# ShreyasBhaktharam/RDEIC

Measured on AMD Instinct MI355X. Metric: 512x512 images/sec encode+relay-decode @ fixed bpp; 1/2/4/8 GPU, higher is better.
Workload: dtype bf16; 1 GPU; config 2: global batch 16 (16/GPU) 512x512, 2-step relay DDIM, encode+entropy-code+decode+VAE-decode; global_batch=16, image_size=512, ddim_steps=2, sampler=ddim, parallelism=dp1, codec_sessions_per_gpu=5

## Files before the change

include/rdeic_hip.h:

```cpp
#ifndef RDEIC_HIP_H
#define RDEIC_HIP_H
#include <stddef.h>
#include <stdint.h>
#ifdef __cplusplus
extern "C" {
#endif

int rdeic_version(void);
int rdeic_abi_count(void);

typedef struct rdeic_conv_desc {
  const void* in0;
  const void* in1;
  int32_t c0, c1;
  int32_t ld0, ld1;
  int32_t n, h, w;
  int32_t up2;
  const void* weight;
  int32_t wld;
  const float* bias;
  int32_t cout, kh, kw, stride, pad_t, pad_l;
  int32_t ho, wo;
  const float* gn_ab;
  int32_t gn_silu;
  const float* emb;
  int32_t emb_ld;
  int32_t act;
  float act_param;
  const void* res;
  int32_t res_ld;
  void* out;
  int32_t out_ld;
  int32_t out_mode;
  int32_t dtype;
  int32_t out_f32;
  int32_t batch;
  int64_t in_bs, w_bs, out_bs;
  float* gn_part;
  int32_t gn_hw;
  int32_t reserved;
  const float* ln_rows;
  const float* ln_colsum;
} rdeic_conv_desc;

int rdeic_conv2d(const rdeic_conv_desc* d, void* stream);
int rdeic_conv2d_tile(const rdeic_conv_desc* d, int32_t tile, void* stream);
int rdeic_conv2d_splitk(const rdeic_conv_desc* d, int32_t splits, float* ws, size_t ws_floats, void* stream);
int rdeic_set_conv_path(int32_t path);
int rdeic_set_conv_option(int32_t key, int32_t value);

size_t rdeic_groupnorm_ws_floats(int32_t n, int32_t hw, int32_t c);
size_t rdeic_groupnorm_parts_floats(int64_t rows, int32_t c, int32_t hw);
int rdeic_groupnorm_parts_ab(const float* p0, int32_t c0, const float* p1, int32_t c1, int32_t n, int32_t hw,
                             int32_t groups, float eps, const float* gamma, const float* beta, float* ab,
                             void* stream);
int rdeic_groupnorm_stats(const void* x0, int32_t c0, int32_t ld0, const void* x1, int32_t c1, int32_t ld1,
                          int32_t n, int32_t hw, int32_t groups, float eps, const float* gamma, const float* beta,
                          float* ab, float* ws, int32_t dtype, void* stream);
int rdeic_groupnorm_parts_apply(const float* p0, int32_t c0, const float* p1, int32_t c1, const void* x0, int32_t ld0,
                                const void* x1, int32_t ld1, int32_t n, int32_t hw, int32_t groups, float eps,
                                const float* gamma, const float* beta, int32_t silu, float* ab, void* y, int32_t yld,
                                void* stream);
int rdeic_groupnorm_apply(const void* x, int32_t n, int32_t hw, int32_t c, int32_t ld, const float* ab,
                          int32_t ab_c, int32_t silu, float out_mul, void* y, int32_t yld, int32_t dtype,
                          void* stream);
int rdeic_layernorm(const void* x, int32_t rows, int32_t c, int32_t ld, const float* gamma, const float* beta,
                    float eps, void* y, int32_t yld, int32_t dtype, void* stream);

int rdeic_attention(const void* q, int32_t ldq, const void* k, int32_t ldk, const void* v, int32_t ldv,
                    void* o, int32_t ldo, int32_t batch, int32_t heads, int32_t lq, int32_t lk, int32_t dh,
                    float scale, int32_t kv_bcast, int32_t dtype, void* stream);
int rdeic_softmax_rows(const float* s, int64_t rows, int32_t cols, float scale, void* p, int32_t dtype, void* stream);
int rdeic_transpose(const void* in, int32_t rows, int32_t cols, int32_t ldin, void* out, int32_t ldout,
                    int32_t batch, int64_t in_bs, int64_t out_bs, int32_t dtype, void* stream);

int rdeic_geglu(const void* in, int32_t rows, int32_t c, int32_t ldin, void* out, int32_t ldout,
                int32_t dtype, void* stream);
int rdeic_nchw_to_nhwc(const float* in, int32_t n, int32_t c, int32_t h, int32_t w, float mul, float add,
                       void* out, int32_t ld, int32_t dtype, void* stream);
int rdeic_nhwc_to_nchw(const void* in, int32_t n, int32_t c, int32_t h, int32_t w, int32_t ld, float mul,
                       float add, float* out, int32_t dtype, void* stream);
int rdeic_axpby(const float* x, const float* z, int32_t n_img, int32_t per_img, const float* a,
                const float* b, float* y, void* stream);
int rdeic_timestep_embedding(const int64_t* t, const float* freqs, int32_t n, int32_t dim, float* out, void* stream);
int rdeic_ddim_step(const float* x, const float* e, int64_t count, float c_sq1m, float c_sqa, float c_sqap,
                    float c_dir, float* xp, float* x0, void* stream);
int rdeic_cfg_combine(const float* e_cond, const float* e_uncond, int64_t count, float scale, float* out,
                      void* stream);
int rdeic_spaced_step(const float* x, const float* e, const float* noise, int64_t count, float a, float b, float c1,
                      float c2, float s, float* xp, float* x0, void* stream);
int rdeic_silu_f32(const float* x, float* y, int64_t count, void* stream);
int rdeic_image_u8_to_nhwc(const uint8_t* img, int32_t n, int32_t h, int32_t w, void* out, int32_t ld,
                           int32_t dtype, void* stream);
int rdeic_nhwc_to_image_u8(const void* x, int32_t n, int32_t h, int32_t w, int32_t ld, uint8_t* img,
                           int32_t dtype, void* stream);
int rdeic_image_mse(const uint8_t* a, const uint8_t* b, int32_t n, int64_t per_img, float* out, void* stream);
int rdeic_fill_uniform(float* out, int64_t count, uint64_t seed, float scale, float offset, void* stream);
int rdeic_pack_conv_weight(const float* w, int32_t cout, int32_t cin, int32_t kh, int32_t kw, void* out,
                           int32_t wld, int32_t dtype, void* stream);
int rdeic_cast(const void* in, int32_t in_dtype, void* out, int32_t out_dtype, int64_t count, void* stream);

int rdeic_ckbd_encode(const void* y, int32_t yld, const void* params, int32_t pld, int32_t n, int32_t hy,
                      int32_t wy, int32_t c, int32_t phase, const float* scale_table, int32_t levels,
                      float scale_bound, int32_t* sym, int32_t* idx, int64_t img_stride, int64_t off,
                      void* yhat, int32_t yhld, void* anchor_out, int32_t ald, int32_t dtype, void* stream);
int rdeic_ckbd_indexes(const void* params, int32_t pld, int32_t n, int32_t hy, int32_t wy, int32_t c,
                       int32_t phase, const float* scale_table, int32_t levels, float scale_bound,
                       int32_t* idx, int64_t img_stride, int64_t off, int32_t dtype, void* stream);
int rdeic_ckbd_dequant(const int32_t* sym, const void* params, int32_t pld, int32_t n, int32_t hy,
                       int32_t wy, int32_t c, int32_t phase, int64_t img_stride, int64_t off, void* yhat,
                       int32_t yhld, void* anchor_out, int32_t ald, int32_t dtype, void* stream);
int rdeic_vq_argmin(const float* dot, const float* zn, const float* en, int32_t rows, int32_t ncode, int32_t* idx,
                    void* stream);
int rdeic_gather_rows(const float* table, int32_t ld_table, const int32_t* idx, int32_t rows, int32_t dim,
                      void* out, int32_t ld_out, int32_t dtype, void* stream);
int rdeic_row_sqnorm(const void* x, int32_t rows, int32_t dim, int32_t ld, float* out, int32_t dtype,
                     void* stream);

size_t rdeic_image_ssim_ws_floats(int32_t n, int32_t h, int32_t w, int32_t levels);
int rdeic_image_ssim(const uint8_t* a, const uint8_t* b, int32_t n, int32_t h, int32_t w, int32_t levels, float* ws,
                     size_t ws_floats, float* out, void* stream);

int rdeic_pmf_to_quantized_cdf(const float* pmf, int32_t n, int32_t precision, uint32_t* cdf_out);
int rdeic_build_gaussian_tables(const float* pmf, const int32_t* pmf_len, int32_t levels, int32_t pmf_ld,
                                int32_t* cdf, int32_t cdf_ld, int32_t* cdf_len, void* reserved);

int rdeic_rans_encode(const int32_t* sym, const int32_t* idx, size_t n, const int32_t* cdf, int32_t cdf_ld,
                      const int32_t* cdf_len, const int32_t* offset, int32_t levels, uint8_t* out, size_t cap,
                      size_t* out_len);
int rdeic_rans_encode_batch(int32_t count, const int32_t* sym, const int32_t* idx, size_t n_per,
                            size_t stride, const int32_t* cdf, int32_t cdf_ld, const int32_t* cdf_len,
                            const int32_t* offset, int32_t levels, uint8_t* out, size_t cap_per,
                            size_t* out_len, int32_t threads);
void* rdeic_rans_enc_tables_create(const int32_t* cdf, int32_t cdf_ld, const int32_t* cdf_len,
                                   const int32_t* offset, int32_t levels);
void rdeic_rans_enc_tables_destroy(void* tables);
int rdeic_rans_encode_batch_t(const void* tables, int32_t count, const int32_t* sym, const int32_t* idx,
                              size_t n_per, size_t stride, uint8_t* out, size_t cap_per, size_t* out_len,
                              int32_t threads);
int rdeic_rans_enc_quotient(const void* tables, int32_t row, int32_t value, uint64_t x, uint64_t* q);
void* rdeic_rans_dec_open(const uint8_t* data, size_t len);
int rdeic_rans_decode(void* handle, const int32_t* idx, size_t n, const int32_t* cdf, int32_t cdf_ld,
                      const int32_t* cdf_len, const int32_t* offset, int32_t levels, int32_t* out);
int rdeic_rans_decode_batch(int32_t count, void** handles, const int32_t* idx, size_t n_per, size_t stride,
                            const int32_t* cdf, int32_t cdf_ld, const int32_t* cdf_len, const int32_t* offset,
                            int32_t levels, int32_t* out, int32_t threads);
void rdeic_rans_dec_close(void* handle);

int rdeic_ac_encode(const int16_t* sym, size_t n, const int16_t* cdf_row, int32_t lp, uint8_t* out,
                    size_t cap, size_t* out_len);
int rdeic_ac_decode(const uint8_t* data, size_t len, size_t n, const int16_t* cdf_row, int32_t lp,
                    int16_t* out);
int rdeic_ac_uniform_cdf(int32_t codebook_size, int16_t* cdf_row);

#define RDEIC_PROF_CONV 0
#define RDEIC_PROF_ATTN 1
#define RDEIC_PROF_ATTN_SMALL 2
#define RDEIC_PROF_GN_STATS 3
#define RDEIC_PROF_GN_APPLY 4
#define RDEIC_PROF_GEMM 5
#define RDEIC_PROF_ATTN_D512 6
#define RDEIC_PROF_CONV_BYTES 7
int rdeic_prof_start(int32_t capacity, int32_t every);
int rdeic_prof_read_keys(int32_t kind, int64_t* keys, int64_t* launches, double* work, double* ms, int32_t cap);
#define RDEIC_COUNT_HALO_CONV 0
#define RDEIC_COUNT_GN_APPLY 1
#define RDEIC_COUNT_LAYERNORM 2
#define RDEIC_COUNT_HALO_SMALL 3
#define RDEIC_COUNT_LN_FUSED 4
#define RDEIC_COUNT_SPLITK 5
#define RDEIC_COUNT_EDGE 6
#define RDEIC_COUNT_GN_PARTS_APPLY 7
#define RDEIC_COUNT_KINDS 8
int64_t rdeic_launch_count(int32_t kind);
int rdeic_layernorm_rowstats(const void* x, int32_t rows, int32_t c, int32_t ld, float eps, float* ms,
                             void* stream);
int rdeic_launch_count_reset(void);
int rdeic_prof_stop(void);
int rdeic_prof_read(int32_t kind, int64_t* launches, double* work, double* ms);

typedef struct rdeic_gemm_desc {
  const void* a;
  int64_t a_bs1, a_bs2, a_sm, a_sk;
  const void* b;
  int64_t b_bs1, b_bs2, b_sk, b_sn;
  void* c;
  int64_t c_bs1, c_bs2, c_sm;
  int32_t batch, nb2, m, n, k, ksplit, dtype, c_f32;
  float alpha, beta;
  float* rsum;
  int64_t rsum_bs;
} rdeic_gemm_desc;
int rdeic_gemm_strided(const rdeic_gemm_desc* d, void* stream);
int rdeic_pack_conv_weight_dgrad(const float* w, int32_t cout, int32_t cin, int32_t kh, int32_t kw, void* out,
                                 int32_t wld, int32_t to_bf16, void* stream);
typedef struct rdeic_pack_job {
  const float* w;
  void* out;
  int64_t start;
  int32_t cout, cin, kh, kw, wld, mode;
// ... 73 lines not shown
```

rdeic_amd/_lib.py:

```python
from __future__ import annotations

import ctypes as C
import os
import threading

_HERE = os.path.dirname(os.path.abspath(__file__))
LIB_PATH = os.environ.get("RDEIC_LIB") or os.path.join(_HERE, "lib", "librdeic_hip.so")

EINVAL, ENOSPC, EBADMSG, ELAUNCH = -22, -28, -74, -5
_ERRNAMES = {EINVAL: "EINVAL (bad argument/shape)", ENOSPC: "ENOSPC (output capacity)",
             EBADMSG: "EBADMSG (corrupt or truncated bitstream)", ELAUNCH: "kernel launch failure"}


class RdeicError(RuntimeError):
    def __init__(self, fn: str, code: int):
        super().__init__(f"{fn} failed: {code} {_ERRNAMES.get(code, '')}")
        self.code = code


class BitstreamError(RdeicError, ValueError):
    """Corrupt / truncated bitstream (the reference's 'decode failure')."""


class ConvDesc(C.Structure):
    _fields_ = [
        ("in0", C.c_void_p), ("in1", C.c_void_p),
        ("c0", C.c_int32), ("c1", C.c_int32), ("ld0", C.c_int32), ("ld1", C.c_int32),
        ("n", C.c_int32), ("h", C.c_int32), ("w", C.c_int32), ("up2", C.c_int32),
        ("weight", C.c_void_p), ("wld", C.c_int32),
        ("bias", C.c_void_p),
        ("cout", C.c_int32), ("kh", C.c_int32), ("kw", C.c_int32), ("stride", C.c_int32),
        ("pad_t", C.c_int32), ("pad_l", C.c_int32),
        ("ho", C.c_int32), ("wo", C.c_int32),
        ("gn_ab", C.c_void_p), ("gn_silu", C.c_int32),
        ("emb", C.c_void_p), ("emb_ld", C.c_int32),
        ("act", C.c_int32), ("act_param", C.c_float),
        ("res", C.c_void_p), ("res_ld", C.c_int32),
        ("out", C.c_void_p), ("out_ld", C.c_int32), ("out_mode", C.c_int32),
        ("dtype", C.c_int32), ("out_f32", C.c_int32),
        ("batch", C.c_int32), ("in_bs", C.c_int64), ("w_bs", C.c_int64), ("out_bs", C.c_int64),
        ("gn_part", C.c_void_p), ("gn_hw", C.c_int32), ("reserved", C.c_int32),
        ("ln_rows", C.c_void_p), ("ln_colsum", C.c_void_p),
    ]


class GemmDesc(C.Structure):
    _fields_ = [
        ("a", C.c_void_p), ("a_bs1", C.c_int64), ("a_bs2", C.c_int64), ("a_sm", C.c_int64), ("a_sk", C.c_int64),
        ("b", C.c_void_p), ("b_bs1", C.c_int64), ("b_bs2", C.c_int64), ("b_sk", C.c_int64), ("b_sn", C.c_int64),
        ("c", C.c_void_p), ("c_bs1", C.c_int64), ("c_bs2", C.c_int64), ("c_sm", C.c_int64),
        ("batch", C.c_int32), ("nb2", C.c_int32), ("m", C.c_int32), ("n", C.c_int32), ("k", C.c_int32),
        ("ksplit", C.c_int32), ("dtype", C.c_int32), ("c_f32", C.c_int32),
        ("alpha", C.c_float), ("beta", C.c_float), ("rsum", C.c_void_p), ("rsum_bs", C.c_int64),
    ]


_p, _i32, _i64, _u64, _f, _sz = C.c_void_p, C.c_int32, C.c_int64, C.c_uint64, C.c_float, C.c_size_t

PROTOTYPES = {
    "rdeic_version": (C.c_int, []),
    "rdeic_abi_count": (C.c_int, []),
    "rdeic_conv2d": (C.c_int, [C.POINTER(ConvDesc), _p]),
    "rdeic_conv2d_splitk": (C.c_int, [C.POINTER(ConvDesc), _i32, _p, C.c_size_t, _p]),
    "rdeic_conv2d_tile": (C.c_int, [C.POINTER(ConvDesc), _i32, _p]),
    "rdeic_prof_start": (C.c_int, [_i32, _i32]),
    "rdeic_prof_stop": (C.c_int, []),
    "rdeic_launch_count": (C.c_int64, [_i32]),
    "rdeic_launch_count_reset": (C.c_int, []),
    "rdeic_layernorm_rowstats": (C.c_int, [C.c_void_p, _i32, _i32, _i32, C.c_float, C.c_void_p, C.c_void_p]),
    "rdeic_prof_read": (C.c_int, [_i32, C.POINTER(C.c_int64), C.POINTER(C.c_double), C.POINTER(C.c_double)]),
    "rdeic_prof_read_keys": (C.c_int, [_i32, C.POINTER(C.c_int64), C.POINTER(C.c_int64), C.POINTER(C.c_double),
                                       C.POINTER(C.c_double), _i32]),
    "rdeic_groupnorm_ws_floats": (_sz, [_i32, _i32, _i32]),
    "rdeic_groupnorm_stats": (C.c_int, [_p, _i32, _i32, _p, _i32, _i32, _i32, _i32, _i32, _f, _p, _p, _p, _p,
                                        _i32, _p]),
    "rdeic_groupnorm_apply": (C.c_int, [_p, _i32, _i32, _i32, _i32, _p, _i32, _i32, _f, _p, _i32, _i32, _p]),
    "rdeic_set_conv_path": (C.c_int, [_i32]),
    "rdeic_set_conv_option": (C.c_int, [_i32, _i32]),
    "rdeic_layernorm": (C.c_int, [_p, _i32, _i32, _i32, _p, _p, _f, _p, _i32, _i32, _p]),
    "rdeic_softmax_rows": (C.c_int, [_p, _i64, _i32, _f, _p, _i32, _p]),
    "rdeic_transpose": (C.c_int, [_p, _i32, _i32, _i32, _p, _i32, _i32, _i64, _i64, _i32, _p]),
    "rdeic_attention": (C.c_int, [_p, _i32, _p, _i32, _p, _i32, _p, _i32, _i32, _i32, _i32, _i32, _i32, _f,
                                  _i32, _i32, _p]),
    "rdeic_geglu": (C.c_int, [_p, _i32, _i32, _i32, _p, _i32, _i32, _p]),
    "rdeic_nchw_to_nhwc": (C.c_int, [_p, _i32, _i32, _i32, _i32, _f, _f, _p, _i32, _i32, _p]),
    "rdeic_nhwc_to_nchw": (C.c_int, [_p, _i32, _i32, _i32, _i32, _i32, _f, _f, _p, _i32, _p]),
    "rdeic_axpby": (C.c_int, [_p, _p, _i32, _i32, _p, _p, _p, _p]),
    "rdeic_timestep_embedding": (C.c_int, [_p, _p, _i32, _i32, _p, _p]),
    "rdeic_ddim_step": (C.c_int, [_p, _p, _i64, _f, _f, _f, _f, _p, _p, _p]),
    "rdeic_spaced_step": (C.c_int, [_p, _p, _p, _i64, _f, _f, _f, _f, _f, _p, _p, _p]),
    "rdeic_cfg_combine": (C.c_int, [_p, _p, _i64, _f, _p, _p]),
    "rdeic_silu_f32": (C.c_int, [_p, _p, _i64, _p]),
    "rdeic_image_u8_to_nhwc": (C.c_int, [_p, _i32, _i32, _i32, _p, _i32, _i32, _p]),
    "rdeic_nhwc_to_image_u8": (C.c_int, [_p, _i32, _i32, _i32, _i32, _p, _i32, _p]),
    "rdeic_image_mse": (C.c_int, [_p, _p, _i32, _i64, _p, _p]),
    "rdeic_fill_uniform": (C.c_int, [_p, _i64, _u64, _f, _f, _p]),
    "rdeic_pack_conv_weight": (C.c_int, [_p, _i32, _i32, _i32, _i32, _p, _i32, _i32, _p]),
    "rdeic_cast": (C.c_int, [_p, _i32, _p, _i32, _i64, _p]),
    "rdeic_ckbd_encode": (C.c_int, [_p, _i32, _p, _i32, _i32, _i32, _i32, _i32, _i32, _p, _i32, _f, _p, _p,
                                    _i64, _i64, _p, _i32, _p, _i32, _i32, _p]),
    "rdeic_ckbd_indexes": (C.c_int, [_p, _i32, _i32, _i32, _i32, _i32, _i32, _p, _i32, _f, _p, _i64, _i64,
                                     _i32, _p]),
    "rdeic_ckbd_dequant": (C.c_int, [_p, _p, _i32, _i32, _i32, _i32, _i32, _i32, _i64, _i64, _p, _i32, _p,
                                     _i32, _i32, _p]),
    "rdeic_vq_argmin": (C.c_int, [_p, _p, _p, _i32, _i32, _p, _p]),
    "rdeic_gather_rows": (C.c_int, [_p, _i32, _p, _i32, _i32, _p, _i32, _i32, _p]),
    "rdeic_row_sqnorm": (C.c_int, [_p, _i32, _i32, _i32, _p, _i32, _p]),
    "rdeic_pmf_to_quantized_cdf": (C.c_int, [_p, _i32, _i32, _p]),
    "rdeic_build_gaussian_tables": (C.c_int, [_p, _p, _i32, _i32, _p, _i32, _p, _p]),
    "rdeic_rans_encode": (C.c_int, [_p, _p, _sz, _p, _i32, _p, _p, _i32, _p, _sz, C.POINTER(_sz)]),
    "rdeic_rans_encode_batch": (C.c_int, [_i32, _p, _p, _sz, _sz, _p, _i32, _p, _p, _i32, _p, _sz, _p, _i32]),
    "rdeic_image_ssim_ws_floats": (C.c_size_t, [_i32, _i32, _i32, _i32]),
    "rdeic_image_ssim": (C.c_int, [_p, _p, _i32, _i32, _i32, _i32, _p, C.c_size_t, _p, _p]),
    "rdeic_groupnorm_parts_floats": (C.c_size_t, [_i64, _i32, _i32]),
    "rdeic_groupnorm_parts_ab": (C.c_int, [_p, _i32, _p, _i32, _i32, _i32, _i32, _f, _p, _p, _p, _p]),
    "rdeic_groupnorm_parts_apply": (C.c_int, [_p, _i32, _p, _i32, _p, _i32, _p, _i32, _i32, _i32, _i32, _f, _p, _p,
                                              _i32, _p, _p, _i32, _p]),
    "rdeic_rans_enc_tables_create": (_p, [_p, _i32, _p, _p, _i32]),
    "rdeic_rans_enc_tables_destroy": (None, [_p]),
    "rdeic_rans_encode_batch_t": (C.c_int, [_p, _i32, _p, _p, _sz, _sz, _p, _sz, _p, _i32]),
    "rdeic_rans_enc_quotient": (C.c_int, [_p, _i32, _i32, C.c_uint64, C.POINTER(C.c_uint64)]),
    "rdeic_rans_dec_open": (_p, [_p, _sz]),
    "rdeic_rans_decode": (C.c_int, [_p, _p, _sz, _p, _i32, _p, _p, _i32, _p]),
    "rdeic_rans_decode_batch": (C.c_int, [_i32, _p, _p, _sz, _sz, _p, _i32, _p, _p, _i32, _p, _i32]),
    "rdeic_rans_dec_close": (None, [_p]),
    "rdeic_ac_encode": (C.c_int, [_p, _sz, _p, _i32, _p, _sz, C.POINTER(_sz)]),
    "rdeic_ac_decode": (C.c_int, [_p, _sz, _sz, _p, _i32, _p]),
    "rdeic_ac_uniform_cdf": (C.c_int, [_i32, _p]),
    "rdeic_gemm_strided": (C.c_int, [C.POINTER(GemmDesc), _p]),
    "rdeic_pack_conv_weight_dgrad": (C.c_int, [_p, _i32, _i32, _i32, _i32, _p, _i32, _i32, _p]),
    "rdeic_pack_batch": (C.c_int, [_p, _i32, _i64, _i32, _i32, _p]),
    "rdeic_zero_insert2": (C.c_int, [_p, _i32, _i32, _i32, _i32, _i32, _p, _i32, _i32, _p]),
    "rdeic_sum_pool2": (C.c_int, [_p, _i32, _i32, _i32, _i32, _i32, _p, _i32, _i32, _p]),
    "rdeic_pixel_unshuffle2": (C.c_int, [_p, _i32, _i32, _i32, _i32, _i32, _p, _i32, _i32, _p]),
    "rdeic_im2col": (C.c_int, [_p, _i32, _i32, _i32, _i32, _i32, _i32, _i32, _i32, _i32, _i32, _i32, _i32, _i32, _p,
                               _i64, _i32, _p]),
    "rdeic_wgrad_finalize": (C.c_int, [_p, _i32, _i32, _i32, _i32, _i32, _p, _i32, _p, _p, _p]),
    "rdeic_col_sum_ws_floats": (_sz, [_i64, _i32, _i32]),
    "rdeic_col_sum": (C.c_int, [_p, _i64, _i32, _i32, _i32, _p, _i32, _p, _sz, _i32, _p]),
    "rdeic_act_fwd": (C.c_int, [_p, _i64, _i32, _i32, _p, _i32, _i32, _f, _p, _i32, _i32, _p]),
    "rdeic_act_bwd": (C.c_int, [_p, _i32, _p, _i32, _i64, _i32, _i32, _f, _p, _i32, _i32, _p]),
    "rdeic_gn_train_ws_doubles": (_sz, [_i32, _i32, _i32]),
    "rdeic_gn_train_fwd": (C.c_int, [_p, _i32, _i32, _i32, _i32, _i32, _f, _p, _p, _p, _p, _p, _i32, _p]),
    "rdeic_gn_train_bwd": (C.c_int, [_p, _i32, _p, _i32, _i32, _i32, _i32, _i32, _p, _p, _p, _i32, _p, _i32, _p, _p,
                                     _i32, _p, _p, _i32, _p]),
    "rdeic_gn_train_bwd_res": (C.c_int, [_p, _i32, _p, _i32, _i32, _i32, _i32, _i32, _p, _p, _p, _i32, _p, _i32, _p,
                                         _i32, _p, _p, _i32, _p, _p, _i32, _p]),
    "rdeic_layernorm_bwd_ws_floats": (_sz, [_i64, _i32]),
    "rdeic_layernorm_bwd": (C.c_int, [_p, _i32, _i64, _i32, _p, _f, _p, _i32, _p, _i32, _p, _p, _i32, _p, _sz, _i32,
                                      _p]),
    "rdeic_layernorm_bwd_res": (C.c_int, [_p, _i32, _i64, _i32, _p, _f, _p, _i32, _p, _i32, _p, _i32, _p, _p, _i32, _p,
                                          _sz, _i32, _p]),
    "rdeic_softmax_bwd_rows": (C.c_int, [_p, _p, _i64, _i32, _f, _p, _i32, _p]),
    "rdeic_geglu_bwd": (C.c_int, [_p, _i32, _i64, _i32, _p, _i32, _p, _i32, _i32, _p]),
    "rdeic_ckbd_train_anchor": (C.c_int, [_p, _i32, _p, _i32, _i32, _i32, _i32, _i32, _p, _i32, _i32, _p]),
    "rdeic_ckbd_mask": (C.c_int, [_p, _i32, _i32, _i32, _i32, _i32, _i32, _p, _i32, _i32, _p]),
    "rdeic_ckbd_train_ws_doubles": (_sz, [_i32, _i32, _i32, _i32]),
    "rdeic_ckbd_train_lik": (C.c_int, [_p, _i32, _p, _i32, _p, _i32, _p, _i32, _i32, _i32, _i32, _p, _i32, _p, _p,
                                       _i32, _p]),
    "rdeic_ckbd_train_lik_bwd": (C.c_int, [_p, _i32, _p, _i32, _p, _i32, _p, _i32, _i32, _i32, _i32, _p, _p, _i32, _p,
                                           _i32, _p, _i32, _p, _i32, _i32, _p]),
    "rdeic_vq_train": (C.c_int, [_p, _p, _p, _p, _p, _i32, _i32, _i32, _p, _p, _f, _f, _f, _p, _p, _p, _p]),
    "rdeic_vq_z_grad": (C.c_int, [_p, _p, _p, _i64, _p, _f, _p, _i32, _p]),
    "rdeic_scale_dev": (C.c_int, [_p, _i64, _p, _p, _i32, _p]),
    "rdeic_adamw": (C.c_int, [_p, _p, _p, _p, _i64, _f, _f, _f, _f, _f, _i32, _p]),
    "rdeic_adamw_dev": (C.c_int, [_p, _p, _p, _p, _i64, _f, _f, _f, _f, _f, _p, _p]),
}

_lib = None
_lock = threading.Lock()


def load() -> C.CDLL:
    global _lib
    if _lib is not None:
        return _lib
    with _lock:
        if _lib is not None:
            return _lib
        if not os.path.exists(LIB_PATH):
            raise ImportError(f"librdeic_hip.so not built at {LIB_PATH}; run `make` (or __graft_entry__.build()).")
        import torch
        lib = C.CDLL(LIB_PATH, mode=C.RTLD_GLOBAL)
        for name, (res, args) in PROTOTYPES.items():
            fn = getattr(lib, name)
            fn.restype = res
            fn.argtypes = args
        _lib = lib
    return _lib


def check(name: str, rc: int) -> None:
    if rc != 0:
        if rc == EBADMSG:
            raise BitstreamError(name, rc)
        raise RdeicError(name, rc)


RECORDER = None


def call(name: str, *args, tag=None) -> None:
    fn = getattr(load(), name)
    if RECORDER is not None:
        RECORDER.append((name, fn, args, tag))
    rc = fn(*args)
    check(name, rc)
```

rdeic_amd/csrc/coders.cpp:

```cpp
#include <stdint.h>
#include <string.h>

#include <algorithm>
#include <atomic>
#include <condition_variable>
#include <functional>
#include <mutex>
#include <cmath>
#include <new>
#include <stdexcept>
#include <thread>
#include <vector>

#include "../../include/rdeic_hip.h"

#define RDEIC_OK 0
#define RDEIC_EINVAL (-22)
#define RDEIC_ENOSPC (-28)
#define RDEIC_EBADMSG (-74)

namespace {

constexpr int kPrecision = 16;
constexpr uint32_t kBypassBits = 4;
// ... 244 lines not shown
  }
  return d->bad ? RDEIC_EBADMSG : RDEIC_OK;
}

class WorkerPool {
 public:
  static WorkerPool& get() {
    thread_local WorkerPool* p = new WorkerPool();
    return *p;
  }
  void run(int32_t count, int32_t threads, const std::function<void(int32_t)>& f) {
    std::lock_guard<std::mutex> job(job_mu_);
    int32_t helpers = std::max(0, std::min(threads, count) - 1);
    while ((int32_t)workers_.size() < helpers) {
      const int32_t id = (int32_t)workers_.size();
      try {
        workers_.reserve(workers_.size() + 1);
        std::thread(&WorkerPool::loop, this, id).detach();
      } catch (...) {
        helpers = (int32_t)workers_.size();
        break;
      }
      workers_.push_back(id);
    }
    {
      std::lock_guard<std::mutex> lk(mu_);
      fn_ = &f;
      count_ = count;
      next_.store(0);
      helpers_ = helpers;
      active_ = helpers;
      ++gen_;
    }
    cv_.notify_all();
    work();
    std::unique_lock<std::mutex> lk(mu_);
    done_cv_.wait(lk, [&] { return active_ == 0; });
    fn_ = nullptr;
  }

 private:
  void work() {
    for (;;) {
      const int32_t i = next_.fetch_add(1);
      if (i >= count_) break;
      (*fn_)(i);
    }
  }
  void loop(int32_t id) {
    uint64_t seen = 0;
    for (;;) {
      {
        std::unique_lock<std::mutex> lk(mu_);
        cv_.wait(lk, [&] { return gen_ != seen; });
        seen = gen_;
        if (id >= helpers_) continue;
      }
      work();
      std::lock_guard<std::mutex> lk(mu_);
      if (--active_ == 0) done_cv_.notify_all();
    }
  }

  std::mutex job_mu_, mu_;
  std::condition_variable cv_, done_cv_;
  std::vector<int32_t> workers_;
  const std::function<void(int32_t)>* fn_ = nullptr;
  std::atomic<int32_t> next_{0};
  int32_t count_ = 0, active_ = 0, helpers_ = 0;
  uint64_t gen_ = 0;
};

template <typename F>
int guard(F&& f) noexcept {
  try {
    return f();
  } catch (const std::bad_alloc&) {
    return RDEIC_ENOSPC;
  } catch (...) {
    return RDEIC_EINVAL;
  }
}

template <typename F>
void parallel_for(int32_t count, int32_t threads, F&& f) {
  if (threads <= 1 || count <= 1) {
    for (int32_t i = 0; i < count; ++i) f(i);
    return;
  }
  const std::function<void(int32_t)> fn = f;
  WorkerPool::get().run(count, threads, fn);
}

struct BitWriter {
  uint8_t* out;
  size_t cap;
  size_t len = 0;
  uint8_t cache = 0;
  int count = 0;
  bool overflow = false;
  void put(int bit) {
    cache = (uint8_t)((cache << 1) | (bit & 1));
    if (++count == 8) {
      if (len < cap) out[len] = cache; else overflow = true;
      ++len;
      count = 0;
      cache = 0;
    }
  }
  void put_with_pending(int bit, uint64_t& pending) {
    put(bit);
    while (pending > 0) { put(!bit); --pending; }
  }
  void flush() {
    while (count > 0) put(0);
  }
};

struct BitReader {
  const uint8_t* in;
  size_t n;
  size_t ptr = 0;
  uint8_t cache = 0;
  int cached = 0;
  void get(uint32_t& value) {
    if (cached == 0) {
      if (ptr == n) { value <<= 1; return; }
      cache = in[ptr++];
      cached = 8;
    }
    value = (value << 1) | ((cache >> (cached - 1)) & 1);
    --cached;
  }
};

inline uint16_t binsearch_u16(const uint16_t* cdf, uint16_t target, uint16_t max_sym) {
  uint16_t left = 0, right = (uint16_t)(max_sym + 1);
  while (left + 1 < right) {
    const uint16_t m = (uint16_t)((left + right) / 2);
    const uint16_t v = cdf[m];
    if (v < target) left = m;
    else if (v > target) right = m;
    else return m;
  }
  return left;
}

}

extern "C" {

int rdeic_version(void) { return 1; }

int rdeic_abi_count(void) { return 93; }

static int pmf_to_quantized_cdf_impl(const float* pmf, int32_t n, int32_t precision, uint32_t* cdf_out) {
  if (!pmf || !cdf_out || n <= 0 || precision <= 0 || precision > 24) return RDEIC_EINVAL;
  for (int32_t i = 0; i < n; ++i)
    if (!(pmf[i] >= 0.f) || !std::isfinite(pmf[i])) return RDEIC_EINVAL;
  const uint32_t one = 1u << precision;
  std::vector<uint32_t> cdf((size_t)n + 1);
  cdf[0] = 0;
  for (int32_t i = 0; i < n; ++i) cdf[i + 1] = (uint32_t)std::round(pmf[i] * (float)one);
  uint64_t total = 0;
  for (uint32_t v : cdf) total += v;
  if (total == 0) return RDEIC_EINVAL;
  for (auto& v : cdf) v = (uint32_t)(((uint64_t)one * v) / total);
  for (size_t i = 1; i < cdf.size(); ++i) cdf[i] += cdf[i - 1];
  cdf.back() = one;
  const int32_t m = (int32_t)cdf.size();
  for (int32_t i = 0; i < m - 1; ++i) {
    if (cdf[i] == cdf[i + 1]) {
      uint32_t best_freq = ~0u;
      int32_t best = -1;
      for (int32_t j = 0; j < m - 1; ++j) {
        const uint32_t f = cdf[j + 1] - cdf[j];
        if (f > 1 && f < best_freq) { best_freq = f; best = j; }
      }
      if (best < 0) return RDEIC_EINVAL;
      if (best < i) {
        for (int32_t j = best + 1; j <= i; ++j) cdf[j]--;
      } else {
        for (int32_t j = i + 1; j <= best; ++j) cdf[j]++;
      }
    }
  }
  memcpy(cdf_out, cdf.data(), cdf.size() * sizeof(uint32_t));
  return RDEIC_OK;
}

int rdeic_pmf_to_quantized_cdf(const float* pmf, int32_t n, int32_t precision, uint32_t* cdf_out) {
  return guard([&] { return pmf_to_quantized_cdf_impl(pmf, n, precision, cdf_out); });
}

static int build_gaussian_tables_impl(const float* pmf, const int32_t* pmf_len, int32_t levels, int32_t pmf_ld,
                                      int32_t* cdf, int32_t cdf_ld, int32_t* cdf_len) {
  if (!pmf || !pmf_len || !cdf || !cdf_len || levels <= 0) return RDEIC_EINVAL;
  std::vector<float> row;
  std::vector<uint32_t> q;
  for (int32_t i = 0; i < levels; ++i) {
    const int32_t L = pmf_len[i];
    if (L <= 0 || L + 1 > pmf_ld || L + 2 > cdf_ld) return RDEIC_EINVAL;
    row.assign(pmf + (size_t)i * pmf_ld, pmf + (size_t)i * pmf_ld + L + 1);
    q.assign((size_t)L + 2, 0u);
    int rc = pmf_to_quantized_cdf_impl(row.data(), L + 1, kPrecision, q.data());
    if (rc) return rc;
    int32_t* out = cdf + (size_t)i * cdf_ld;
    for (int32_t j = 0; j < cdf_ld; ++j) out[j] = j < L + 2 ? (int32_t)q[j] : 0;
    cdf_len[i] = L + 2;
  }
  return RDEIC_OK;
}

int rdeic_build_gaussian_tables(const float* pmf, const int32_t* pmf_len, int32_t levels, int32_t pmf_ld, int32_t* cdf,
                                int32_t cdf_ld, int32_t* cdf_len, void* reserved) {
  (void)reserved;
  return guard([&] { return build_gaussian_tables_impl(pmf, pmf_len, levels, pmf_ld, cdf, cdf_ld, cdf_len); });
}

int rdeic_rans_encode(const int32_t* sym, const int32_t* idx, size_t n, const int32_t* cdf, int32_t cdf_ld,
                      const int32_t* cdf_len, const int32_t* offset, int32_t levels, uint8_t* out, size_t cap,
                      size_t* out_len) {
  if ((!sym || !idx) && n) return RDEIC_EINVAL;
  if (!cdf || !cdf_len || !offset || !out || !out_len || levels <= 0) return RDEIC_EINVAL;
  return guard([&] {
    std::vector<RansSym> syms;
    std::vector<uint32_t> words;
    return rans_encode_impl(sym, idx, n, cdf, cdf_ld, cdf_len, offset, levels, out, cap, out_len, syms, words);
  });
}

int rdeic_rans_encode_batch(int32_t count, const int32_t* sym, const int32_t* idx, size_t n_per, size_t stride,
                            const int32_t* cdf, int32_t cdf_ld, const int32_t* cdf_len, const int32_t* offset,
                            int32_t levels, uint8_t* out, size_t cap_per, size_t* out_len, int32_t threads) {
  if (count <= 0 || !sym || !idx || !out || !out_len) return RDEIC_EINVAL;
  return guard([&] {
    std::vector<int> rc(count, 0);
    parallel_for(count, threads, [&](int32_t i) {
      rc[i] = guard([&] {
        std::vector<RansSym> syms;
        std::vector<uint32_t> words;
        return rans_encode_impl(sym + i * stride, idx + i * stride, n_per, cdf, cdf_ld, cdf_len, offset, levels,
                                out + i * cap_per, cap_per, &out_len[i], syms, words);
      });
    });
    for (int v : rc)
      if (v) return v;
    return (int)RDEIC_OK;
  });
}

void* rdeic_rans_enc_tables_create(const int32_t* cdf, int32_t cdf_ld, const int32_t* cdf_len, const int32_t* offset,
                                   int32_t levels) {
  if (!cdf || !cdf_len || !offset || levels <= 0 || cdf_ld < 2) return nullptr;
  EncTables* T = new (std::nothrow) EncTables();
  if (!T) return nullptr;
  try {
    T->levels = levels;
    T->row_off.resize(levels);
    T->max_value.resize(levels);
    T->offset.assign(offset, offset + levels);
    size_t total = 0;
    for (int32_t ci = 0; ci < levels; ++ci) {
      const int32_t len = cdf_len[ci];
      if (len < 2 || len > cdf_ld) throw std::invalid_argument("cdf_len");
      T->row_off[ci] = (int32_t)total;
      T->max_value[ci] = len - 2;
      total += (size_t)len - 1;
    }
    T->sym.resize(total);
    for (int32_t ci = 0; ci < levels; ++ci) {
      const int32_t* row = cdf + (size_t)ci * cdf_ld;
      for (int32_t v = 0; v <= T->max_value[ci]; ++v) {
        const int32_t start = row[v], freq = row[v + 1] - row[v];
        if (start < 0 || freq <= 0 || start + freq > (1 << kPrecision)) throw std::invalid_argument("cdf row");
        T->sym[(size_t)T->row_off[ci] + v] = make_enc_sym((uint32_t)start, (uint32_t)freq);
      }
    }
  } catch (...) {
    delete T;
    return nullptr;
  }
  return T;
}

void rdeic_rans_enc_tables_destroy(void* tables) { delete (EncTables*)tables; }

int rdeic_rans_encode_batch_t(const void* tables, int32_t count, const int32_t* sym, const int32_t* idx, size_t n_per,
                              size_t stride, uint8_t* out, size_t cap_per, size_t* out_len, int32_t threads) {
  if (!tables || count <= 0 || ((!sym || !idx) && n_per) || !out || !out_len) return RDEIC_EINVAL;
  const EncTables& T = *(const EncTables*)tables;
  return guard([&] {
    std::vector<int> rc(count, 0);
    parallel_for(count, threads, [&](int32_t i) {
      rc[i] = guard([&] {
        thread_local std::vector<uint32_t> buf;
        return rans_encode_tab_impl(T, sym + i * stride, idx + i * stride, n_per, out + i * cap_per, cap_per,
                                    &out_len[i], buf);
      });
    });
    for (int v : rc)
      if (v) return v;
    return (int)RDEIC_OK;
  });
}

int rdeic_rans_enc_quotient(const void* tables, int32_t row, int32_t value, uint64_t x, uint64_t* q) {
// ... 151 lines not shown
```

rdeic_amd/csrc/conv_common.h:

```cpp
#pragma once
#include "common.h"
#include "../../include/rdeic_hip.h"
#include "prof.h"

namespace rdeic_conv {

struct ConvArgs {
  const char* in0; const char* in1;
  int c0, c1, ld0, ld1;
  int n, h, w, up2;
  const char* weight; int wld;
  const float* bias;
  int cout, kh, kw, stride, pad_t, pad_l, ho, wo;
  const float* gn_ab; int gn_silu;
  const float* emb; int emb_ld;
  int act; float act_param;
  const char* res; int res_ld;
  char* out; int out_ld, out_mode;
  int out_f32;
  int M, cin, ktot, nk;
  long in_bs, w_bs, out_bs;
  int batch;
  int epi_vec;
  int splits, kper;
  float* gn_part;
  int gn_row0;
  int gn_hw;
  const float* ln_rows;
  const float* ln_cs;
};

__device__ __forceinline__ float ln_fold(const ConvArgs& a, int m, int n, float v) {
  const float2 ms = reinterpret_cast<const float2*>(a.ln_rows)[m];
  return ms.y * (v - ms.x * a.ln_cs[n]);
}

constexpr int ROWB = 144;

template <typename T, bool SWZ = true> __host__ __device__ constexpr int tile_rowb() { return (sizeof(T) == 2 && SWZ) ? 128 : ROWB; }
template <typename T, bool SWZ = true> __device__ __forceinline__ int chunk_key(int r) {
  if constexpr (sizeof(T) == 2 && SWZ) return (((r >> 3) & 1) << 1) | (((r >> 1) & 1) << 2);
  return 0;
}
template <typename T, int BM, int BN, bool SWZ = true> __host__ __device__ constexpr int conv_lds_bytes() {
  return (2 * (BM + BN) * tile_rowb<T, SWZ>() > (BM / 2) * (BN + 4) * 4 || sizeof(T) != 2)
             ? 2 * (BM + BN) * tile_rowb<T, SWZ>()
             : (BM / 2) * (BN + 4) * 4;
}

template <typename T> struct MmaTraits;
template <> struct MmaTraits<bf16> {
  static constexpr int BK = 64;
  static constexpr int EPC = 8;
};
template <> struct MmaTraits<float> {
  static constexpr int BK = 32;
  static constexpr int EPC = 4;
};

__device__ __forceinline__ float apply_act(float v, int act, float p) {
  if (act == 1) return v >= 0.f ? v : v * p;
  if (act == 2) return gelu_f(v);
  if (act == 3) return silu_f(v);
  return v;
}

__device__ __forceinline__ uint4 ld16(const char* p) { return *reinterpret_cast<const uint4*>(p); }

template <typename T>
__device__ __forceinline__ uint4 gn_apply_chunk(uint4 raw, const float* ab, int silu) {
  constexpr int E = MmaTraits<T>::EPC;
  T v[E];
  *reinterpret_cast<uint4*>(v) = raw;
#pragma unroll
  for (int e = 0; e < E; ++e) {
    float x = to_f32(v[e]);
    x = x * ab[2 * e] + ab[2 * e + 1];
    if (silu) x = silu_f(x);
    v[e] = from_f32<T>(x);
  }
  return *reinterpret_cast<uint4*>(v);
}

__host__ __device__ __forceinline__ bool epi_vec_ok(const ConvArgs& a) {
  if (a.out_mode == 2) return (a.cout % 8) == 0 && (a.out_ld % 4) == 0 && ((uintptr_t)a.out % 8) == 0;
  return a.out_mode == 0 && (a.cout % 8) == 0 && (a.out_ld % 8) == 0 && ((uintptr_t)a.out % 16) == 0 &&
         (!a.res || ((a.res_ld % 8) == 0 && ((uintptr_t)a.res % 16) == 0));
}

struct RowsFrom {
  int m0;
  __device__ __forceinline__ int operator()(int r) const { return m0 + r; }
};

template <int BM, int BN, int WGM, int WGN, int NT, int P = 2, class RowMap = RowsFrom, bool PF = true>
__device__ __forceinline__ void epilogue_vec(const f32x4 (&acc)[BM / WGM / 16][BN / WGN / 16], const ConvArgs& a,
                                             int m0, int n0, int wm, int wn, int lane, int tid, char* lds,
                                             RowMap rmap = RowMap{0}) {
  if constexpr (__is_same(RowMap, RowsFrom)) rmap.m0 = m0;
  constexpr int WTM = BM / WGM, WTN = BN / WGN;
  constexpr int TM = WTM / 16, TN = WTN / 16;
  constexpr int HM = TM / P;
  constexpr int PR = BM / P;
  constexpr int SDW = BN + 4;
  constexpr int CPR = BN / 8;
  static_assert(TM % P == 0, "P passes");
  const int lr = lane & 15, lq = lane >> 4;
  float* L = reinterpret_cast<float*>(lds);
  const int hw_o = a.ho * a.wo;
  const bool of32 = a.out_f32;
  const bool st = a.gn_part != nullptr;
  constexpr int NU = ((BM / 64) * BN + NT - 1) / NT;
  float sg[NU][4], qg[NU][4];
#pragma unroll
  for (int u = 0; u < NU; ++u)
#pragma unroll
    for (int g = 0; g < 4; ++g) sg[u][g] = qg[u][g] = 0.f;
  constexpr int NCH = (PR * CPR + NT - 1) / NT;
  constexpr int NPF = !PF ? 0 : NCH < 2 ? NCH : 2;
  constexpr bool HOIST = PF && (NT % CPR) == 0;
  auto bar = []() { asm volatile("s_waitcnt lgkmcnt(0)\n\ts_barrier" ::: "memory"); };
  float4 bh[2] = {float4{0.f, 0.f, 0.f, 0.f}, float4{0.f, 0.f, 0.f, 0.f}}, chh[2] = {bh[0], bh[0]};
  if constexpr (HOIST) {
    const int nn = n0 + (tid % CPR) * 8;
    if (nn < a.cout) {
      if (a.bias) {
        bh[0] = *reinterpret_cast<const float4*>(a.bias + nn);
        bh[1] = *reinterpret_cast<const float4*>(a.bias + nn + 4);
      }
      if (a.ln_rows) {
        chh[0] = *reinterpret_cast<const float4*>(a.ln_cs + nn);
        chh[1] = *reinterpret_cast<const float4*>(a.ln_cs + nn + 4);
      }
    }
  }
#pragma unroll
  for (int p = 0; p < P; ++p) {
    uint4 rpf[NPF > 0 ? NPF : 1];
    float2 lpf[NPF > 0 ? NPF : 1];
#pragma unroll
    for (int k = 0; k < NPF; ++k) {
      const int c = tid + k * NT;
      const int pr = c / CPR, cc = c - pr * CPR;
      const int wmr = pr / (WTM / P), wr = pr - wmr * (WTM / P);
      const int m = rmap(wmr * WTM + p * (WTM / P) + wr);
      const int nn = n0 + cc * 8;
      const bool ok = c < PR * CPR && m < a.M && nn < a.cout;
      rpf[k] = uint4{0u, 0u, 0u, 0u};
      lpf[k] = float2{0.f, 0.f};
      if (ok) {
        if (a.res && !of32 && a.out_mode != 2)
          rpf[k] = *reinterpret_cast<const uint4*>(reinterpret_cast<const bf16*>(a.res) + (long)m * a.res_ld + nn);
        if (a.ln_rows) lpf[k] = reinterpret_cast<const float2*>(a.ln_rows)[m];
      }
    }
    bar();
#pragma unroll
    for (int ii = 0; ii < HM; ++ii)
#pragma unroll
      for (int r = 0; r < 4; ++r) {
        const int pr = wm * (WTM / P) + ii * 16 + lq * 4 + r;
#pragma unroll
        for (int j = 0; j < TN; ++j) L[pr * SDW + wn * WTN + j * 16 + lr] = acc[p * HM + ii][j][r];
      }
    bar();
#pragma unroll
    for (int k = 0; k < NCH; ++k) {
      const int c = tid + k * NT;
      if (c >= PR * CPR) continue;
      const int pr = c / CPR, cc = c - pr * CPR;
      const int wmr = pr / (WTM / P), wr = pr - wmr * (WTM / P);
      const int m = rmap(wmr * WTM + p * (WTM / P) + wr);
      const int nn = n0 + cc * 8;
      if (m >= a.M || nn >= a.cout) continue;
      float v[8];
      const float4 x0 = *reinterpret_cast<const float4*>(L + pr * SDW + cc * 8);
      const float4 x1 = *reinterpret_cast<const float4*>(L + pr * SDW + cc * 8 + 4);
      v[0] = x0.x; v[1] = x0.y; v[2] = x0.z; v[3] = x0.w; v[4] = x1.x; v[5] = x1.y; v[6] = x1.z; v[7] = x1.w;
      if (a.ln_rows) {
        const float2 ms = k < NPF ? lpf[k < NPF ? k : 0] : reinterpret_cast<const float2*>(a.ln_rows)[m];
        float4 c0 = chh[0], c1 = chh[1];
        if constexpr (!HOIST) {
          c0 = *reinterpret_cast<const float4*>(a.ln_cs + nn);
          c1 = *reinterpret_cast<const float4*>(a.ln_cs + nn + 4);
        }
        const float cs[8] = {c0.x, c0.y, c0.z, c0.w, c1.x, c1.y, c1.z, c1.w};
        const f32x2 nm = {-ms.x, -ms.x}, rs = {ms.y, ms.y};
#pragma unroll
        for (int e = 0; e < 8; e += 2) {
          const f32x2 r = rs * pk_fma(nm, f32x2{cs[e], cs[e + 1]}, f32x2{v[e], v[e + 1]});
          v[e] = r.x;
          v[e + 1] = r.y;
        }
      }
      if (a.bias) {
        float4 b0 = bh[0], b1 = bh[1];
        if constexpr (!HOIST) {
          b0 = *reinterpret_cast<const float4*>(a.bias + nn);
          b1 = *reinterpret_cast<const float4*>(a.bias + nn + 4);
        }
        const float bs[8] = {b0.x, b0.y, b0.z, b0.w, b1.x, b1.y, b1.z, b1.w};
#pragma unroll
        for (int e = 0; e < 8; e += 2) {
          const f32x2 r = f32x2{v[e], v[e + 1]} + f32x2{bs[e], bs[e + 1]};
          v[e] = r.x;
          v[e + 1] = r.y;
        }
      }
      if (a.emb) {
        const float* em = a.emb + (long)(m / hw_o) * a.emb_ld + nn;
#pragma unroll
        for (int e = 0; e < 8; ++e) v[e] += em[e];
      }
#pragma unroll
      for (int e = 0; e < 8; ++e) v[e] = apply_act(v[e], a.act, a.act_param);
      if (a.out_mode == 2) {
        bf16 gv[4];
#pragma unroll
        for (int e = 0; e < 4; e += 2) {
          const f32x2 xv = {to_f32(from_f32<bf16>(v[e])), to_f32(from_f32<bf16>(v[e + 1]))};
          const f32x2 gt = {to_f32(from_f32<bf16>(v[4 + e])), to_f32(from_f32<bf16>(v[5 + e]))};
          const f32x2 r = xv * gelu_fast2(gt);
          gv[e] = from_f32<bf16>(r.x);
          gv[e + 1] = from_f32<bf16>(r.y);
        }
        *reinterpret_cast<uint2*>(reinterpret_cast<bf16*>(a.out) + (long)m * a.out_ld + (nn >> 1)) =
            *reinterpret_cast<uint2*>(gv);
        continue;
      }
      if (a.res) {
        if (of32) {
          const float4 r0 = *reinterpret_cast<const float4*>(reinterpret_cast<const float*>(a.res) + (long)m * a.res_ld + nn);
          const float4 r1 = *reinterpret_cast<const float4*>(reinterpret_cast<const float*>(a.res) + (long)m * a.res_ld + nn + 4);
          v[0] += r0.x; v[1] += r0.y; v[2] += r0.z; v[3] += r0.w; v[4] += r1.x; v[5] += r1.y; v[6] += r1.z; v[7] += r1.w;
        } else {
          bf16 rv[8];
          *reinterpret_cast<uint4*>(rv) =
              k < NPF ? rpf[k < NPF ? k : 0]
                      : *reinterpret_cast<const uint4*>(reinterpret_cast<const bf16*>(a.res) + (long)m * a.res_ld + nn);
#pragma unroll
          for (int e = 0; e < 8; ++e) v[e] += to_f32(rv[e]);
        }
      }
      if (of32) {
        float* o = reinterpret_cast<float*>(a.out) + (long)m * a.out_ld + nn;
        *reinterpret_cast<float4*>(o) = make_float4(v[0], v[1], v[2], v[3]);
        *reinterpret_cast<float4*>(o + 4) = make_float4(v[4], v[5], v[6], v[7]);
        if (st) {
          *reinterpret_cast<float4*>(L + pr * SDW + cc * 8) = make_float4(v[0], v[1], v[2], v[3]);
          *reinterpret_cast<float4*>(L + pr * SDW + cc * 8 + 4) = make_float4(v[4], v[5], v[6], v[7]);
        }
      } else {
        bf16 ov[8];
#pragma unroll
        for (int e = 0; e < 8; ++e) ov[e] = from_f32<bf16>(v[e]);
        *reinterpret_cast<uint4*>(reinterpret_cast<bf16*>(a.out) + (long)m * a.out_ld + nn) = *reinterpret_cast<uint4*>(ov);
        if (st) {
          *reinterpret_cast<float4*>(L + pr * SDW + cc * 8) =
              make_float4(to_f32(ov[0]), to_f32(ov[1]), to_f32(ov[2]), to_f32(ov[3]));
          *reinterpret_cast<float4*>(L + pr * SDW + cc * 8 + 4) =
              make_float4(to_f32(ov[4]), to_f32(ov[5]), to_f32(ov[6]), to_f32(ov[7]));
        }
      }
    }
    if constexpr ((WTM == 32 || WTM == 64) && (WTM / P) % 16 == 0) {
      if (st) {
        bar();
#pragma unroll
        for (int u = 0; u < NU; ++u) {
        const int b = (tid + u * NT) / BN, j = (tid + u * NT) % BN;
        if (b < BM / 64) {
          constexpr int WPB = 64 / WTM;
#pragma unroll
          for (int w = 0; w < WPB; ++w) {
            const int wmr = b * WPB + w;
#pragma unroll
            for (int k = 0; k < (WTM / P) / 16; ++k) {
              const int off = w * WTM + p * (WTM / P) + k * 16;
              const float* col = L + (wmr * (WTM / P) + k * 16) * SDW + j;
              const int nv = a.M - (rmap(b * 64) + off);
              float s1 = 0.f, s2 = 0.f;
              if (nv >= 16) {
                float y[16];
#pragma unroll
                for (int r = 0; r < 16; ++r) y[r] = col[r * SDW];
#pragma unroll
                for (int r = 0; r < 16; ++r) { s1 += y[r]; s2 = fmaf(y[r], y[r], s2); }
              } else {
                for (int r = 0; r < nv; ++r) { const float y = col[r * SDW]; s1 += y; s2 = fmaf(y, y, s2); }
              }
              sg[u][off >> 4] = s1;
              qg[u][off >> 4] = s2;
            }
          }
        }
        }
      }
    }
  }
  if constexpr ((WTM == 32 || WTM == 64) && (WTM / P) % 16 == 0) {
    if (st) {
#pragma unroll
      for (int u = 0; u < NU; ++u) {
        const int b = (tid + u * NT) / BN, j = (tid + u * NT) % BN;
        const int nn = n0 + j;
        if (b < BM / 64 && nn < a.cout && rmap(b * 64) < a.M) {
          float* pp = a.gn_part + 4 + ((long)((a.gn_row0 + rmap(b * 64)) / 64) * a.cout + nn) * 2;
          pp[0] = ((sg[u][0] + sg[u][1]) + sg[u][2]) + sg[u][3];
          pp[1] = ((qg[u][0] + qg[u][1]) + qg[u][2]) + qg[u][3];
        }
      }
      if (tid == 0 && rmap(0) == 0 && n0 == 0) reinterpret_cast<int*>(a.gn_part)[0] = 64;
    }
  }
}

template <int BM, int BN, int WGM, int NT, int P>
constexpr bool stats_tile_ok() {
  constexpr int WTM = BM / WGM;
  return (WTM == 32 || WTM == 64) && (WTM / P) % 16 == 0;
}

template <int BM, int BN, int WGM, int WGN, int NT, int P>
__device__ __forceinline__ void epilogue_geglu(const f32x4 (&acc)[BM / WGM / 16][BN / WGN / 16], const ConvArgs& a,
                                               int m0, int n0, int wm, int wn, int lane, int tid, char* lds) {
  constexpr int WTM = BM / WGM, WTN = BN / WGN;
  constexpr int TM = WTM / 16, TN = WTN / 16;
  constexpr int HM = TM / P;
  constexpr int PR = BM / P;
  constexpr int SDW = BN + 4;
  constexpr int DPR = BN / 16;
  constexpr int ND = (PR * DPR + NT - 1) / NT;
  constexpr int NPF = ND < 2 ? ND : 2;
  constexpr bool HOIST = (NT % DPR) == 0;
  static_assert(TM % P == 0 && BN % 16 == 0, "P passes, chunk pairs");
  const int lr = lane & 15, lq = lane >> 4;
  float* L = reinterpret_cast<float*>(lds);
  auto bar = []() { asm volatile("s_waitcnt lgkmcnt(0)\n\ts_barrier" ::: "memory"); };
  auto row_of = [&](int d, int p) {
    const int pr = d / DPR;
    const int wmr = pr / (WTM / P), wr = pr - wmr * (WTM / P);
    return m0 + wmr * WTM + p * (WTM / P) + wr;
  };
  float4 bh[4], chh[4];
#pragma unroll
  for (int q = 0; q < 4; ++q) bh[q] = chh[q] = float4{0.f, 0.f, 0.f, 0.f};
  if constexpr (HOIST) {
    const int nn = n0 + (tid % DPR) * 16;
    if (nn < a.cout) {
#pragma unroll
      for (int q = 0; q < 4; ++q) {
        if (a.bias) bh[q] = *reinterpret_cast<const float4*>(a.bias + nn + 4 * q);
        if (a.ln_rows) chh[q] = *reinterpret_cast<const float4*>(a.ln_cs + nn + 4 * q);
      }
    }
  }
#pragma unroll
  for (int p = 0; p < P; ++p) {
    float2 lpf[NPF];
#pragma unroll
    for (int k = 0; k < NPF; ++k) {
      const int d = tid + k * NT;
      const int m = row_of(d, p);
      lpf[k] = float2{0.f, 0.f};
      if (a.ln_rows && d < PR * DPR && m < a.M) lpf[k] = reinterpret_cast<const float2*>(a.ln_rows)[m];
    }
    bar();
#pragma unroll
    for (int ii = 0; ii < HM; ++ii)
#pragma unroll
      for (int r = 0; r < 4; ++r) {
        const int pr = wm * (WTM / P) + ii * 16 + lq * 4 + r;
#pragma unroll
        for (int j = 0; j < TN; ++j) L[pr * SDW + wn * WTN + j * 16 + lr] = acc[p * HM + ii][j][r];
      }
    bar();
#pragma unroll
    for (int k = 0; k < ND; ++k) {
      const int d = tid + k * NT;
      if (d >= PR * DPR) continue;
      const int pr = d / DPR, cq = d - pr * DPR;
      const int m = row_of(d, p);
      const int nn = n0 + cq * 16;
      if (m >= a.M || nn >= a.cout) continue;
      float v[16];
#pragma unroll
      for (int q = 0; q < 4; ++q) {
        const float4 x = *reinterpret_cast<const float4*>(L + pr * SDW + cq * 16 + 4 * q);
        v[4 * q] = x.x; v[4 * q + 1] = x.y; v[4 * q + 2] = x.z; v[4 * q + 3] = x.w;
      }
      if (a.ln_rows) {
        const float2 ms = k < NPF ? lpf[k < NPF ? k : 0] : reinterpret_cast<const float2*>(a.ln_rows)[m];
        const f32x2 nm = {-ms.x, -ms.x}, rs = {ms.y, ms.y};
#pragma unroll
        for (int q = 0; q < 4; ++q) {
          const float4 c = HOIST ? chh[q] : *reinterpret_cast<const float4*>(a.ln_cs + nn + 4 * q);
          const float cs[4] = {c.x, c.y, c.z, c.w};
#pragma unroll
          for (int e = 0; e < 4; e += 2) {
            const f32x2 r = rs * pk_fma(nm, f32x2{cs[e], cs[e + 1]}, f32x2{v[4 * q + e], v[4 * q + e + 1]});
            v[4 * q + e] = r.x;
            v[4 * q + e + 1] = r.y;
          }
        }
      }
      if (a.bias) {
#pragma unroll
        for (int q = 0; q < 4; ++q) {
          const float4 b = HOIST ? bh[q] : *reinterpret_cast<const float4*>(a.bias + nn + 4 * q);
          const f32x2 r0 = f32x2{v[4 * q], v[4 * q + 1]} + f32x2{b.x, b.y};
          const f32x2 r1 = f32x2{v[4 * q + 2], v[4 * q + 3]} + f32x2{b.z, b.w};
          v[4 * q] = r0.x; v[4 * q + 1] = r0.y; v[4 * q + 2] = r1.x; v[4 * q + 3] = r1.y;
        }
      }
#pragma unroll
      for (int e = 0; e < 16; ++e) v[e] = apply_act(v[e], a.act, a.act_param);
      bf16 gv[8];
#pragma unroll
      for (int h = 0; h < 2; ++h)
#pragma unroll
        for (int e = 0; e < 4; e += 2) {
          const f32x2 xv = {to_f32(from_f32<bf16>(v[8 * h + e])), to_f32(from_f32<bf16>(v[8 * h + e + 1]))};
          const f32x2 gt = {to_f32(from_f32<bf16>(v[8 * h + 4 + e])), to_f32(from_f32<bf16>(v[8 * h + 5 + e]))};
          const f32x2 r = xv * gelu_fast2(gt);
          gv[4 * h + e] = from_f32<bf16>(r.x);
          gv[4 * h + e + 1] = from_f32<bf16>(r.y);
        }
      *reinterpret_cast<uint4*>(reinterpret_cast<bf16*>(a.out) + (long)m * a.out_ld + (nn >> 1)) =
          *reinterpret_cast<uint4*>(gv);
    }
  }
}

constexpr unsigned kOOB = 0x80000000u;

template <int N>
__device__ __forceinline__ void wait_vm() {
  asm volatile("s_waitcnt vmcnt(%0)" ::"n"(N) : "memory");
}

__device__ __forceinline__ int dma_key(int r) { return (((r >> 3) & 1) << 1) | (((r >> 1) & 1) << 2); }

typedef __attribute__((address_space(3))) void* lds_ptr_t;

__device__ __forceinline__ void dma16(__amdgpu_buffer_rsrc_t rs, char* lds_dst, unsigned voff, int soff) {
  __builtin_amdgcn_raw_ptr_buffer_load_lds(rs, (lds_ptr_t)lds_dst, 16, (int)voff, soff, 0, 0);
}

#ifdef RDEIC_HALO_STAMPS
__device__ unsigned long long* g_halo_stamps;
#define HALO_STAMP(k)                                                                      \
  do {                                                                                     \
    if (threadIdx.x == 0) g_halo_stamps[(long)blockIdx.x * 8 + (k)] = __builtin_amdgcn_s_memtime(); \
  } while (0)
#else
#define HALO_STAMP(k) do {} while (0)
#endif

__device__ __forceinline__ void wait_vm_rt(int n) {
  switch (n) {
    case 0: wait_vm<0>(); break;
    case 1: wait_vm<1>(); break;
    case 2: wait_vm<2>(); break;
    case 3: wait_vm<3>(); break;
    case 4: wait_vm<4>(); break;
    case 5: wait_vm<5>(); break;
    case 6: wait_vm<6>(); break;
    default: wait_vm<7>(); break;
  }
}

extern int g_conv_path, g_epi_vec, g_swz, g_force_tile, g_dma, g_halo, g_halo8, g_edge;

int make_args(const rdeic_conv_desc* d, ConvArgs& a, bool& vec);
bool dma_ok(const rdeic_conv_desc* d, const ConvArgs& a, unsigned& b0, unsigned& b1, unsigned& bw);
int launch_dma_auto(const ConvArgs& a, unsigned b0, unsigned b1, unsigned bw, hipStream_t s, int tile,
                    int gn_hw = 0, bool* fused = nullptr);
int dma_grouped(const rdeic_conv_desc* d, int tile, hipStream_t s, bool* fused = nullptr);
bool halo_ok(const rdeic_conv_desc* d, const ConvArgs& a);
int launch_halo(const rdeic_conv_desc* d, ConvArgs a, hipStream_t s, bool* fused);
int launch_edge(const rdeic_conv_desc* d, const ConvArgs& a, hipStream_t s, bool* fused);
}
```

rdeic_amd/csrc/conv_dma.hip:

```cpp
#include "conv_common.h"

namespace rdeic_conv {

template <int TM, int TN, int WTM, int WTN>
__device__ __forceinline__ void epilogue_scalar(const f32x4 (&acc)[TM][TN], const ConvArgs& a, int m0, int n0, int wm,
                                                int wn, int lane) {
  if (a.out_mode == 2) return;
  const int lrow = lane & 15, lq = lane >> 4;
  const int hw_o = a.ho * a.wo;
  const bool of32 = a.out_f32;
#pragma unroll
  for (int i = 0; i < TM; ++i) {
#pragma unroll
    for (int r = 0; r < 4; ++r) {
      const int m = m0 + wm * WTM + i * 16 + lq * 4 + r;
      if (m >= a.M) continue;
      const int img = m / hw_o;
      int oy = 0, ox = 0;
      if (a.out_mode == 1) { const int rem = m - img * hw_o; oy = rem / a.wo; ox = rem - oy * a.wo; }
#pragma unroll
      for (int j = 0; j < TN; ++j) {
        const int nn = n0 + wn * WTN + j * 16 + lrow;
        if (nn >= a.cout) continue;
        float v = acc[i][j][r];
        if (a.ln_rows) v = ln_fold(a, m, nn, v);
        if (a.bias) v += a.bias[nn];
        if (a.emb) v += a.emb[(long)img * a.emb_ld + nn];
        v = apply_act(v, a.act, a.act_param);
        long oidx, ridx;
        if (a.out_mode == 1) {
          const int c = nn >> 2, dy = (nn >> 1) & 1, dx = nn & 1;
          const long p = ((long)img * (2 * a.ho) + (2 * oy + dy)) * (2 * a.wo) + (2 * ox + dx);
          oidx = p * a.out_ld + c;
          ridx = p * a.res_ld + c;
        } else {
          oidx = (long)m * a.out_ld + nn;
          ridx = (long)m * a.res_ld + nn;
        }
        if (a.res) v += of32 ? reinterpret_cast<const float*>(a.res)[ridx] : to_f32(reinterpret_cast<const bf16*>(a.res)[ridx]);
        if (of32) reinterpret_cast<float*>(a.out)[oidx] = v;
        else reinterpret_cast<bf16*>(a.out)[oidx] = from_f32<bf16>(v);
      }
    }
  }
}

template <int BM, int BN, int WGM, int WGN, int S, int EP, bool GEG = false>
__device__ __forceinline__ void conv_dma_body(ConvArgs a, int tiles_n, unsigned bytes0, unsigned bytes1,
                                              unsigned bytesw) {
  constexpr int KB = 64;
  constexpr int NW = WGM * WGN, NT = NW * 64;
  constexpr int RB = KB * 2;
  constexpr int RPI = 1024 / RB;
  constexpr int LPR = RB / 16;
  constexpr int KSUB = KB / 32;
  constexpr int A_BYTES = BM * RB, STAGE = (BM + BN) * RB;
  constexpr int AI = BM / NW / RPI, BI = BN / NW / RPI;
  constexpr int PER = AI + BI;
  constexpr int WTM = BM / WGM, WTN = BN / WGN;
  constexpr int TM = WTM / 16, TN = WTN / 16;
  static_assert(AI >= 1 && BI >= 1 && AI * RPI * NW == BM && BI * RPI * NW == BN, "tile / wave split");
  static_assert(S >= 2 && S <= 4 && PER * (S - 2) <= 63, "ring");

  extern __shared__ __attribute__((aligned(16))) char lds[];
  HALO_STAMP(0);

  int kt_begin = 0, kt_end = a.nk;
  if (a.splits > 1) {
    const int z = blockIdx.z;
    kt_begin = min(a.nk, z * a.kper);
    kt_end = min(a.nk, kt_begin + a.kper);
    a.out += (long)z * a.M * a.out_ld * 4;
  } else if (gridDim.z > 1) {
    const long z = blockIdx.z;
    a.in0 += z * a.in_bs * 2; a.in1 += z * a.in_bs * 2;
    a.weight += z * a.w_bs * 2;
    a.out += z * a.out_bs * (a.out_f32 ? 4 : 2);
  }
  const int nwg = gridDim.x, orig = blockIdx.x;
  const int xcd = orig & 7, q = nwg >> 3, rr = nwg & 7;
  const int wgid = (xcd < rr ? xcd * (q + 1) : rr * (q + 1) + (xcd - rr) * q) + (orig >> 3);
  const int mt = wgid / tiles_n, nt = wgid - mt * tiles_n;
  const int m0 = mt * BM, n0 = nt * BN;

  const int tid = threadIdx.x, lane = tid & 63;
  const int wave = __builtin_amdgcn_readfirstlane(tid >> 6);
  const int wm = wave / WGN, wn = wave - (wave / WGN) * WGN;
  const int g = lane / LPR, sl = lane % LPR;
  const int ce = sl ^ (((g >> 1) & 1) << 2);
  const int hw_o = a.ho * a.wo;
  const int hin = a.up2 ? 2 * a.h : a.h, win = a.up2 ? 2 * a.w : a.w;

  const __amdgpu_buffer_rsrc_t rs0 = __builtin_amdgcn_make_buffer_rsrc((void*)a.in0, (short)0, (int)bytes0, 0x00020000);
  const __amdgpu_buffer_rsrc_t rs1 = __builtin_amdgcn_make_buffer_rsrc((void*)a.in1, (short)0, (int)bytes1, 0x00020000);
  const __amdgpu_buffer_rsrc_t rsw = __builtin_amdgcn_make_buffer_rsrc((void*)a.weight, (short)0, (int)bytesw, 0x00020000);

  int r_img[AI], r_iy[AI], r_ix[AI], pix[AI];
  unsigned voa[AI];
#pragma unroll
  for (int j = 0; j < AI; ++j) {
    const int m = m0 + (wave * AI + j) * RPI + g;
    if (m < a.M) {
      const int img = m / hw_o, rem = m - img * hw_o;
      const int oy = rem / a.wo, ox = rem - oy * a.wo;
      r_img[j] = img;
      r_iy[j] = oy * a.stride - a.pad_t;
      r_ix[j] = ox * a.stride - a.pad_l;
    } else {
      r_img[j] = -1; r_iy[j] = 0; r_ix[j] = 0;
    }
  }
  unsigned vob[BI];
#pragma unroll
  for (int j = 0; j < BI; ++j) {
    const int nn = n0 + (wave * BI + j) * RPI + g;
    const int ch = ce ^ (((wave * BI + j) & 1) << 1);
    vob[j] = nn < a.cout ? (unsigned)nn * (unsigned)(a.wld * 2) + ch * 16 : kOOB;
  }

  const int nb0 = a.c0 / KB, nb1 = a.c1 / KB;
  int i_tap = kt_begin / (nb0 + nb1), i_seg = 0, i_cb = kt_begin - i_tap * (nb0 + nb1);
  if (i_cb >= nb0) { i_seg = 1; i_cb -= nb0; }
  auto set_rows = [&]() {
    const int ky = i_tap / a.kw, kx = i_tap - (i_tap / a.kw) * a.kw;
#pragma unroll
    for (int j = 0; j < AI; ++j) {
      int iy = r_iy[j] + ky, ix = r_ix[j] + kx;
      const bool ok = r_img[j] >= 0 && (unsigned)iy < (unsigned)hin && (unsigned)ix < (unsigned)win;
      if (a.up2) { iy >>= 1; ix >>= 1; }
      pix[j] = ok ? (r_img[j] * a.h + iy) * a.w + ix : -1;
    }
  };
  auto set_voff = [&]() {
    const unsigned ldb = (unsigned)(i_seg ? a.ld1 : a.ld0) * 2u;
#pragma unroll
    for (int j = 0; j < AI; ++j) {
      const int ch = ce ^ (((wave * AI + j) & 1) << 1);
      voa[j] = pix[j] >= 0 ? (unsigned)pix[j] * ldb + ch * 16 : kOOB;
    }
  };
  set_rows();
  set_voff();

  auto issue = [&](int kt, int slot) {
    char* sb = lds + slot * STAGE;
    const __amdgpu_buffer_rsrc_t rsa = i_seg ? rs1 : rs0;
    const int soa = i_cb * RB;
#pragma unroll
    for (int j = 0; j < AI; ++j)
      dma16(rsa, sb + (wave * AI + j) * 1024, voa[j], soa);
#pragma unroll
    for (int j = 0; j < BI; ++j) dma16(rsw, sb + A_BYTES + (wave * BI + j) * 1024, vob[j], kt * RB);
    if (++i_cb == (i_seg ? nb1 : nb0)) {
      i_cb = 0;
      if (i_seg == 0 && nb1 > 0) {
        i_seg = 1;
      } else {
        i_seg = 0;
        ++i_tap;
        if (i_tap < a.kh * a.kw) set_rows();
      }
      set_voff();
    }
  };

  f32x4 acc[TM][TN];
#pragma unroll
  for (int i = 0; i < TM; ++i)
#pragma unroll
    for (int j = 0; j < TN; ++j) acc[i][j] = f32x4{0.f, 0.f, 0.f, 0.f};

  const int lrow = lane & 15, lq = lane >> 4;
  const int rkey = dma_key(lrow);
  const int nk = kt_end - kt_begin;

#pragma unroll
  for (int s = 0; s < S - 1; ++s)
    if (s < nk) issue(kt_begin + s, s);
  HALO_STAMP(1);

  for (int t = 0; t < nk; ++t) {
    if constexpr (S == 2) {
      wait_vm<0>();
    } else if constexpr (S == 3) {
      if (t + 1 < nk) wait_vm<PER>(); else wait_vm<0>();
    } else {
      if (t + 2 < nk) wait_vm<2 * PER>(); else if (t + 1 < nk) wait_vm<PER>(); else wait_vm<0>();
    }
    __builtin_amdgcn_s_barrier();
    if (t + S - 1 < nk) issue(kt_begin + t + S - 1, (t + S - 1) % S);
    const int cur = t % S;
    const char* Ab = lds + cur * STAGE + (wm * WTM + lrow) * RB;
    const char* Bb = lds + cur * STAGE + A_BYTES + (wn * WTN + lrow) * RB;
#pragma unroll
    for (int s = 0; s < KSUB; ++s) {
      const int so = ((s * 4 + lq) ^ rkey) * 16;
      bf16x8 bfv[TN];
#pragma unroll
      for (int j = 0; j < TN; ++j) bfv[j] = *reinterpret_cast<const bf16x8*>(Bb + j * 16 * RB + so);
#pragma unroll
      for (int i = 0; i < TM; ++i) {
        const bf16x8 af = *reinterpret_cast<const bf16x8*>(Ab + i * 16 * RB + so);
#pragma unroll
        for (int j = 0; j < TN; ++j) acc[i][j] = __builtin_amdgcn_mfma_f32_16x16x32_bf16(af, bfv[j], acc[i][j], 0, 0, 0);
      }
    }
  }

  HALO_STAMP(2);
  if constexpr (TM % EP == 0 && (BM / EP) * (BN + 4) * 4 <= S * STAGE) {
    if ((a.epi_vec || a.out_mode == 2) && epi_vec_ok(a)) {
      if constexpr (GEG) epilogue_geglu<BM, BN, WGM, WGN, NT, EP>(acc, a, m0, n0, wm, wn, lane, tid, lds);
      else epilogue_vec<BM, BN, WGM, WGN, NT, EP>(acc, a, m0, n0, wm, wn, lane, tid, lds);
      HALO_STAMP(3);
      return;
    }
  }
  epilogue_scalar<TM, TN, WTM, WTN>(acc, a, m0, n0, wm, wn, lane);
  HALO_STAMP(3);
}

template <int BM, int BN, int WGM, int WGN, int S, int EP, bool GEG = false>
__global__ __launch_bounds__(WGM * WGN * 64) void conv_dma_kernel(ConvArgs a, int tiles_n, unsigned bytes0,
                                                                  unsigned bytes1, unsigned bytesw) {
  conv_dma_body<BM, BN, WGM, WGN, S, EP, GEG>(a, tiles_n, bytes0, bytes1, bytesw);
}

template <int BM, int BN, int WGM, int WGN, int S, int EP, bool GEG = false>
__global__ __launch_bounds__(WGM * WGN * 64) __attribute__((amdgpu_num_sgpr(80))) void conv_dma_kernel_2pc(
    ConvArgs a, int tiles_n, unsigned bytes0, unsigned bytes1, unsigned bytesw) {
  conv_dma_body<BM, BN, WGM, WGN, S, EP, GEG>(a, tiles_n, bytes0, bytes1, bytesw);
}

bool dma_ok(const rdeic_conv_desc* d, const ConvArgs& a, unsigned& b0, unsigned& b1, unsigned& bw) {
  if (d->dtype != 1 || d->gn_ab || (d->c0 % 64) || (d->c1 % 64) || (d->ld0 % 8) || ((uintptr_t)d->in0 % 16)) return false;
  if (d->c1 && ((d->ld1 % 8) || ((uintptr_t)d->in1 % 16))) return false;
  if (d->wld % 64 || a.ktot % 64) return false;
  const long pix = (long)d->n * d->h * d->w;
  const long e0 = ((pix - 1) * d->ld0 + d->c0) * 2 + (a.batch - 1) * d->in_bs * 2;
  const long e1 = d->c1 ? ((pix - 1) * d->ld1 + d->c1) * 2 : 16;
  const long ew = (long)d->cout * d->wld * 2 + (a.batch - 1) * d->w_bs * 2;
  if (e0 >= (1l << 31) || e1 >= (1l << 31) || ew >= (1l << 31)) return false;
  if (a.batch > 1 && (d->in_bs % 8 || d->w_bs % 8)) return false;
  b0 = (unsigned)(((pix - 1) * d->ld0 + d->c0) * 2);
  b1 = (unsigned)e1;
  bw = (unsigned)((long)d->cout * d->wld * 2);
  return true;
}

namespace {
template <int BM, int BN, int WGM, int WGN, int S, int EP>
bool dma_vec_epilogue(const ConvArgs& a) {
  constexpr int TM = BM / WGM / 16;
  constexpr bool fits = TM % EP == 0 && (BM / EP) * (BN + 4) * 4 <= S * (BM + BN) * 128;
  return fits && (a.epi_vec || a.out_mode == 2) && epi_vec_ok(a);
}

template <int BM, int BN, int WGM, int WGN, int S, int EP>
int launch_dma(ConvArgs a, unsigned b0, unsigned b1, unsigned bw, hipStream_t s, int gn_hw, bool* fused) {
  if (a.gn_part) {
    const bool ok = a.splits <= 1 && a.batch == 1 && a.out_mode == 0 && gn_hw > 0 && gn_hw % 64 == 0 &&
                    stats_tile_ok<BM, BN, WGM, WGM * WGN * 64, EP>() && dma_vec_epilogue<BM, BN, WGM, WGN, S, EP>(a);
    if (!ok) a.gn_part = nullptr;
    if (fused) *fused = ok;
  }
  const int tn = cdiv(a.cout, BN);
  const long tiles = (long)cdiv(a.M, BM) * tn;
  dim3 grid((unsigned)tiles, 1, a.splits > 1 ? a.splits : a.batch);
  constexpr int lds = S * (BM + BN) * 128;
  const bool geg = a.out_mode == 2 && a.cout % 16 == 0 && a.out_ld % 8 == 0 && ((uintptr_t)a.out % 16) == 0 &&
                   dma_vec_epilogue<BM, BN, WGM, WGN, S, EP>(a);
  if constexpr (WGM * WGN == 16 && lds <= 80 * 1024) {
    hipLaunchKernelGGL((conv_dma_kernel_2pc<BM, BN, WGM, WGN, S, EP>), grid, dim3(WGM * WGN * 64), lds, s, a, tn, b0,
                       b1, bw);
  } else {
    if (geg)
      hipLaunchKernelGGL((conv_dma_kernel<BM, BN, WGM, WGN, S, EP, true>), grid, dim3(WGM * WGN * 64), lds, s, a, tn,
                         b0, b1, bw);
    else
      hipLaunchKernelGGL((conv_dma_kernel<BM, BN, WGM, WGN, S, EP>), grid, dim3(WGM * WGN * 64), lds, s, a, tn, b0, b1,
                         bw);
  }
  return launch_status();
}
}

int launch_dma_auto(const ConvArgs& a, unsigned b0, unsigned b1, unsigned bw, hipStream_t s, int tile, int gn_hw,
                    bool* fused) {
  if (tile < 21 || tile > 38) {
    const long zb = a.splits > 1 ? a.splits : a.batch;
    const long t128 = (long)cdiv(a.M, 128) * cdiv(a.cout, 128) * zb;
    const long t256 = (long)cdiv(a.M, 256) * cdiv(a.cout, 256) * zb;
    const float useful256 = (float)a.M * a.cout / ((float)cdiv(a.M, 256) * 256 * cdiv(a.cout, 256) * 256);
    tile = (t256 >= 256 && useful256 >= 0.9f) ? 32 : t128 >= 256 ? 25 : 26;
  }
  switch (tile) {
    case 21: return launch_dma<256, 128, 4, 2, 3, 2>(a, b0, b1, bw, s, gn_hw, fused);
    case 22: return launch_dma<128, 256, 2, 4, 3, 2>(a, b0, b1, bw, s, gn_hw, fused);
    case 24: return launch_dma<128, 128, 2, 2, 2, 2>(a, b0, b1, bw, s, gn_hw, fused);
    case 25: return launch_dma<128, 128, 2, 4, 2, 2>(a, b0, b1, bw, s, gn_hw, fused);
    case 26: return launch_dma<64, 128, 2, 2, 3, 2>(a, b0, b1, bw, s, gn_hw, fused);
    case 27: return launch_dma<128, 128, 2, 4, 3, 2>(a, b0, b1, bw, s, gn_hw, fused);
    case 28: return launch_dma<256, 128, 4, 2, 2, 2>(a, b0, b1, bw, s, gn_hw, fused);
    case 29: return launch_dma<128, 256, 2, 4, 2, 2>(a, b0, b1, bw, s, gn_hw, fused);
    case 30: return launch_dma<64, 128, 2, 2, 2, 2>(a, b0, b1, bw, s, gn_hw, fused);
    case 31: return launch_dma<128, 64, 2, 2, 2, 2>(a, b0, b1, bw, s, gn_hw, fused);
    case 32: return launch_dma<256, 256, 4, 4, 2, 4>(a, b0, b1, bw, s, gn_hw, fused);
    case 33: return launch_dma<256, 128, 4, 4, 2, 2>(a, b0, b1, bw, s, gn_hw, fused);
    case 34: return launch_dma<128, 128, 4, 4, 2, 2>(a, b0, b1, bw, s, gn_hw, fused);
    case 35: return launch_dma<512, 128, 8, 2, 2, 2>(a, b0, b1, bw, s, gn_hw, fused);
    case 36: return launch_dma<64, 128, 2, 4, 2, 2>(a, b0, b1, bw, s, gn_hw, fused);
    case 37: return launch_dma<128, 160, 2, 2, 2, 2>(a, b0, b1, bw, s, gn_hw, fused);
    case 38: return launch_dma<64, 160, 2, 2, 2, 2>(a, b0, b1, bw, s, gn_hw, fused);
    default: return launch_dma<128, 128, 2, 2, 3, 2>(a, b0, b1, bw, s, gn_hw, fused);
  }
}

int dma_grouped(const rdeic_conv_desc* d, int tile, hipStream_t s, bool* fused) {
  ConvArgs a;
  bool vec = false;
  if (make_args(d, a, vec) != RDEIC_OK || !vec) return -1;
  unsigned b0, b1, bw;
  if (dma_ok(d, a, b0, b1, bw)) return launch_dma_auto(a, b0, b1, bw, s, tile, d->gn_hw, fused);
  if (d->batch > 1 || d->n <= 1) return -1;
  const long ipix = (long)d->h * d->w;
  const long per0 = ipix * d->ld0 * 2, per1 = d->c1 ? ipix * d->ld1 * 2 : 0;
  const long per = per0 > per1 ? per0 : per1;
  const int g = (int)(((1l << 31) - 1) / per);
  if (g < 1) return -1;
  rdeic_conv_desc e = *d;
  const int osz = (d->out_f32 || d->dtype == 0) ? 4 : 2;
  const long opix = d->out_mode == 1 ? 4l * d->ho * d->wo : (long)d->ho * d->wo;
  for (int i0 = 0; i0 < d->n; i0 += g) {
    e.n = d->n - i0 < g ? d->n - i0 : g;
    e.in0 = (const char*)d->in0 + i0 * per0;
    e.in1 = d->in1 ? (const char*)d->in1 + i0 * per1 : nullptr;
    e.out = (char*)d->out + i0 * opix * d->out_ld * osz;
    e.res = d->res ? (const char*)d->res + i0 * opix * d->res_ld * osz : nullptr;
    e.emb = d->emb ? d->emb + (long)i0 * d->emb_ld : nullptr;
    e.ln_rows = d->ln_rows ? d->ln_rows + 2l * i0 * d->ho * d->wo : nullptr;
    ConvArgs ea;
    if (make_args(&e, ea, vec) != RDEIC_OK || !vec || !dma_ok(&e, ea, b0, b1, bw)) return -1;
    ea.gn_row0 = i0 * d->ho * d->wo;
    bool f = false;
    const int rc = launch_dma_auto(ea, b0, b1, bw, s, tile, d->gn_hw, &f);
    if (rc != RDEIC_OK) return rc;
    if (fused) *fused = (i0 == 0 ? f : (*fused && f));
  }
  return RDEIC_OK;
}

}
```

rdeic_amd/csrc/conv_gemm.hip:

```cpp
#include "conv_common.h"

namespace rdeic_conv {

int g_conv_path = 2;
int g_epi_vec = 1;
int g_swz = 1;
int g_force_tile = -1;
int g_dma = 1;
int g_halo = 1;
int g_halo8 = 1;

namespace {

template <typename T, int BM, int BN, int WGM, int WGN, bool VEC, bool GNP = true, bool SWZ = true>
__global__ __launch_bounds__(WGM * WGN * 64) void conv_kernel(ConvArgs a) {
  constexpr int NT = WGM * WGN * 64;
  constexpr int BK = MmaTraits<T>::BK;
  constexpr int EPC = MmaTraits<T>::EPC;
  constexpr int ES = sizeof(T);
  constexpr int WTM = BM / WGM, WTN = BN / WGN;
  constexpr int TM = WTM / 16, TN = WTN / 16;
  constexpr int RPI = NT / 8;
  constexpr int AR = BM / RPI;
  constexpr int BR = (BN + RPI - 1) / RPI;
  static_assert(TM >= 1 && TN >= 1 && AR >= 1 && BM % RPI == 0, "tile");

  extern __shared__ __attribute__((aligned(16))) char lds[];
  constexpr int RB = tile_rowb<T, SWZ>();
#define AS(b) (lds + (b) * (BM + BN) * RB)
#define BS(b) (lds + (b) * (BM + BN) * RB + BM * RB)

  int kt_begin = 0, kt_end = a.nk;
  if (a.splits > 1) {
    const int z = blockIdx.z;
    kt_begin = min(a.nk, z * a.kper);
    kt_end = min(a.nk, kt_begin + a.kper);
    a.out += (long)z * a.M * a.out_ld * 4;
  } else if (gridDim.z > 1) {
    const long z = blockIdx.z;
    a.in0 += z * a.in_bs * ES; a.in1 += z * a.in_bs * ES;
    a.weight += z * a.w_bs * ES;
    a.out += z * a.out_bs * (((sizeof(T) == 4) || a.out_f32) ? 4 : ES);
  }
  const int tid = threadIdx.x;
  const int lane = tid & 63, wave = tid >> 6;
  const int wm = wave / WGN, wn = wave % WGN;
  const int m0 = blockIdx.x * BM, n0 = blockIdx.y * BN;
  const int kc = tid & 7;
  const int hw_o = a.ho * a.wo;
  const int hin = a.up2 ? 2 * a.h : a.h, win = a.up2 ? 2 * a.w : a.w;

  int r_img[AR], r_iy[AR], r_ix[AR];
#pragma unroll
  for (int i = 0; i < AR; ++i) {
    int m = m0 + (tid >> 3) + RPI * i;
    if (m < a.M) {
      int img = m / hw_o, rem = m - img * hw_o;
      int oy = rem / a.wo, ox = rem - oy * a.wo;
      r_img[i] = img;
      r_iy[i] = oy * a.stride - a.pad_t;
      r_ix[i] = ox * a.stride - a.pad_l;
    } else {
      r_img[i] = -1; r_iy[i] = 0; r_ix[i] = 0;
    }
  }

  uint4 areg[AR];
  uint4 breg[BR];
  int a_c[AR];

  auto gather_a = [&](int kt, uint4 (&areg)[AR]) {
    const int k0 = kt * BK + kc * EPC;
    if constexpr (VEC) {
      bool kval = k0 < a.ktot;
      int tap = kval ? k0 / a.cin : 0;
      int c = k0 - tap * a.cin;
      int ky = tap / a.kw, kx = tap - ky * a.kw;
      const char* base; int ld, cs;
      if (c < a.c0) { base = a.in0; ld = a.ld0; cs = c; } else { base = a.in1; ld = a.ld1; cs = c - a.c0; }
#pragma unroll
      for (int i = 0; i < AR; ++i) {
        int iy = r_iy[i] + ky, ix = r_ix[i] + kx;
        bool ok = kval && r_img[i] >= 0 && iy >= 0 && iy < hin && ix >= 0 && ix < win;
        if (ok) {
          if (a.up2) { iy >>= 1; ix >>= 1; }
          long pix = ((long)r_img[i] * a.h + iy) * a.w + ix;
          areg[i] = ld16(base + (pix * ld + cs) * ES);
          a_c[i] = c;
        } else {
          areg[i] = make_uint4(0, 0, 0, 0);
          a_c[i] = -1;
        }
      }
    } else {
#pragma unroll
      for (int i = 0; i < AR; ++i) {
        T v[EPC];
#pragma unroll
        for (int e = 0; e < EPC; ++e) {
          int k = k0 + e;
          float x = 0.f;
          if (k < a.ktot && r_img[i] >= 0) {
            int tap = k / a.cin, c = k - tap * a.cin;
            int ky = tap / a.kw, kx = tap - ky * a.kw;
            int iy = r_iy[i] + ky, ix = r_ix[i] + kx;
            if (iy >= 0 && iy < hin && ix >= 0 && ix < win) {
              if (a.up2) { iy >>= 1; ix >>= 1; }
              long pix = ((long)r_img[i] * a.h + iy) * a.w + ix;
              const T* src = (c < a.c0) ? reinterpret_cast<const T*>(a.in0) + pix * a.ld0 + c
                                        : reinterpret_cast<const T*>(a.in1) + pix * a.ld1 + (c - a.c0);
              x = to_f32(*src);
              if (GNP && a.gn_ab) {
                const float* ab = a.gn_ab + ((long)r_img[i] * a.cin + c) * 2;
                x = x * ab[0] + ab[1];
                if (a.gn_silu) x = silu_f(x);
              }
            }
          }
          v[e] = from_f32<T>(x);
        }
        areg[i] = *reinterpret_cast<uint4*>(v);
        a_c[i] = -1;
      }
    }
  };

  auto gather_b = [&](int kt, uint4 (&breg)[BR]) {
#pragma unroll
    for (int i = 0; i < BR; ++i) {
      int cid = tid + NT * i;
      int row = cid >> 3, ch = cid & 7;
      if (row < BN) {
        int nn = n0 + row;
        if (nn < a.cout)
          breg[i] = ld16(a.weight + ((long)nn * a.wld + kt * BK + ch * EPC) * ES);
        else
          breg[i] = make_uint4(0, 0, 0, 0);
      }
    }
  };

  auto store_tiles = [&](int buf, const uint4 (&areg)[AR], const uint4 (&breg)[BR]) {
#pragma unroll
    for (int i = 0; i < AR; ++i) {
      uint4 v = areg[i];
      if constexpr (VEC) {
        if (GNP && a.gn_ab && a_c[i] >= 0)
          v = gn_apply_chunk<T>(v, a.gn_ab + ((long)r_img[i] * a.cin + a_c[i]) * 2, a.gn_silu);
      }
      int row = (tid >> 3) + RPI * i;
      *reinterpret_cast<uint4*>(AS(buf) + row * RB + (kc ^ chunk_key<T, SWZ>(row)) * 16) = v;
    }
#pragma unroll
    for (int i = 0; i < BR; ++i) {
      int cid = tid + NT * i;
      int row = cid >> 3, ch = cid & 7;
      if (row < BN) *reinterpret_cast<uint4*>(BS(buf) + row * RB + (ch ^ chunk_key<T, SWZ>(row)) * 16) = breg[i];
    }
  };

  f32x4 acc[TM][TN];
#pragma unroll
  for (int i = 0; i < TM; ++i)
// ... 406 lines not shown
    if (d->cout <= 32) return launch_cfg<bf16, 128, 32, 4, 1>(a, vec, s);
    if (d->cout % 128 != 0 && d->cout % 64 == 0) return launch_cfg<bf16, 128, 64, 2, 2>(a, vec, s);
    if (a.M <= 4096) return launch_cfg<bf16, 64, 128, 2, 2>(a, vec, s);
    return launch_cfg<bf16, 128, 128, 2, 2>(a, vec, s);
  } else {
    if (d->cout <= 16) return launch_cfg<float, 64, 16, 4, 1>(a, vec, s);
    if (d->cout >= 128 && (long)cdiv(a.M, 128) * cdiv(a.cout, 128) * a.batch >= 512)
      return launch_cfg<float, 128, 128, 2, 2>(a, vec, s);
    return launch_cfg<float, 64, 64, 2, 2>(a, vec, s);
  }
}

static int conv2d_tile_run(const rdeic_conv_desc* d, int32_t tile, void* stream, bool* fused) {
  ConvArgs a;
  bool vec = false;
  const int rc = make_args(d, a, vec);
  if (rc != RDEIC_OK) return rc;
  if (vec) {
    const int rc2 = launch_edge(d, a, (hipStream_t)stream, fused);
    if (rc2 != -1) return rc2;
  }
  if (d->out_mode == 2) {
    const int rc2 = vec ? dma_grouped(d, tile >= 20 ? tile : -1, (hipStream_t)stream) : -1;
    return rc2 == -1 ? RDEIC_EINVAL : rc2;
  }
  if (d->dtype == 1 && vec && !d->gn_ab && d->cout > 32 && g_conv_path != 0) {
    if (tile >= 20) {
      const int rc2 = dma_grouped(d, tile, (hipStream_t)stream, fused);
      if (rc2 != -1) return rc2;
      tile = -1;
    }
    return launch_plain_auto(a, (hipStream_t)stream, tile, fused);
  }
  return conv2d_run(d, stream, fused);
}

static double conv_flops(const rdeic_conv_desc* d) {
  if (!d) return 0.0;
  const double b = d->batch > 1 ? d->batch : 1;
  return 2.0 * b * d->n * d->ho * d->wo * d->cout * (double)d->kh * d->kw * (d->c0 + d->c1);
}

static double conv_bytes(const rdeic_conv_desc* d) {
  if (!d) return 0.0;
  const double b = d->batch > 1 ? d->batch : 1;
  const double es = d->dtype == 1 ? 2.0 : 4.0, os = (d->dtype == 0 || d->out_f32) ? 4.0 : 2.0;
  const double in = b * d->n * (double)d->h * d->w * (d->c0 + d->c1) * es;
  const double w = (double)(d->batch > 1 ? b : 1) * d->cout * d->wld * es;
  double outc = d->out_mode == 2 ? d->cout / 2.0 : (double)d->cout;
  const double out = b * d->n * (d->out_mode == 1 ? 4.0 : 1.0) * d->ho * d->wo * (d->out_mode == 1 ? outc / 4 : outc) * os;
  return in + w + out + (d->res ? out : 0.0);
}

static int conv2d_impl(const rdeic_conv_desc* d, int32_t tile, void* stream) {
  if (d && d->gn_part &&
      (d->gn_hw <= 0 || d->gn_hw % 64 || d->batch > 1 || d->out_mode != 0 || (long)d->n * d->ho * d->wo % d->gn_hw))
    return RDEIC_EINVAL;
  bool fused = false;
  int rc;
  {
    rdeic_prof_add_bytes(conv_bytes(d));
    ProfScope ps((hipStream_t)stream, RDEIC_PROF_CONV, conv_flops(d));
    rc = tile == -2 ? conv2d_run(d, stream, &fused) : conv2d_tile_run(d, tile, stream, &fused);
  }
  if (rc != RDEIC_OK || !d->gn_part || fused) return rc;
  const long rows = (long)d->n * d->ho * d->wo;
  return gn_rows_partial(d->out, rows, d->cout, d->out_ld, d->gn_hw, d->gn_part,
                         (d->out_f32 || d->dtype == 0) ? 0 : 1, (hipStream_t)stream);
}

static int conv2d_splitk_impl(const rdeic_conv_desc* d, int32_t splits, float* ws, size_t ws_floats,
                              void* stream) {
  ConvArgs a;
  bool vec = false;
  const int rc = make_args(d, a, vec);
  if (rc != RDEIC_OK) return rc;
  if (!vec || d->gn_ab || d->out_mode != 0 || a.batch != 1 || d->cout % 8 || splits < 2 || !ws ||
      (d->out_ld % 8) || ((uintptr_t)d->out % 16) || ((uintptr_t)ws % 16))
    return RDEIC_EINVAL;
  if (ws_floats < (size_t)splits * a.M * a.cout) return RDEIC_ENOSPC;
  hipStream_t s = (hipStream_t)stream;
  float* const part = ws;
  if (d->dtype == 0) {
    ConvArgs p = a;
    p.bias = nullptr; p.emb = nullptr; p.act = 0; p.res = nullptr; p.gn_part = nullptr; p.ln_rows = nullptr;
    p.out = (char*)part; p.out_ld = a.cout; p.out_f32 = 0;
    p.splits = splits;
    p.kper = (a.nk + splits - 1) / splits;
    dim3 grid(cdiv(a.M, 64), cdiv(a.cout, 64), splits);
    constexpr int lds = conv_lds_bytes<float, 64, 64>();
    hipLaunchKernelGGL((conv_kernel<float, 64, 64, 2, 2, true, false, true>), grid, dim3(256), lds, s, p);
    a.splits = splits;
    a.out_f32 = 1;
    const long chunks = (long)a.M * (a.cout / 8);
    hipLaunchKernelGGL(splitk_reduce_kernel, dim3((unsigned)((chunks + 255) / 256)), dim3(256), 0, s, a,
                       (const float*)part);
    return launch_status();
  }
  if (g_dma) {
    rdeic_conv_desc e = *d;
    e.bias = nullptr; e.emb = nullptr; e.act = 0; e.res = nullptr; e.gn_part = nullptr; e.ln_rows = nullptr;
    e.out = part; e.out_ld = d->cout; e.out_f32 = 1;
    ConvArgs pa;
    bool pv = false;
    unsigned b0, b1, bw;
    if (make_args(&e, pa, pv) == RDEIC_OK && pv && dma_ok(&e, pa, b0, b1, bw)) {
      pa.splits = splits; pa.kper = (pa.nk + splits - 1) / splits;
      if (launch_dma_auto(pa, b0, b1, bw, s, -1) == RDEIC_OK) {
        a.splits = splits;
        const long chunks = (long)a.M * (a.cout / 8);
        hipLaunchKernelGGL(splitk_reduce_kernel, dim3((unsigned)((chunks + 255) / 256)), dim3(256), 0, s, a,
                           (const float*)part);
        return launch_status();
      }
    }
  }
  ConvArgs p = a;
  p.bias = nullptr; p.emb = nullptr; p.act = 0; p.res = nullptr; p.gn_part = nullptr; p.ln_rows = nullptr;
  p.out = (char*)part; p.out_ld = a.cout; p.out_f32 = 1;
  p.splits = splits;
  p.kper = (a.nk + splits - 1) / splits;
  dim3 grid(cdiv(a.M, 128), cdiv(a.cout, 128), splits);
  constexpr int lds = conv_lds_bytes<bf16, 128, 128>();
  hipLaunchKernelGGL((conv_kernel<bf16, 128, 128, 2, 2, true, false, true>), grid, dim3(256), lds, s, p);
  a.splits = splits;
  const long chunks = (long)a.M * (a.cout / 8);
  hipLaunchKernelGGL(splitk_reduce_kernel, dim3((unsigned)((chunks + 255) / 256)), dim3(256), 0, s, a,
                     (const float*)part);
  return launch_status();
}

extern "C" int rdeic_conv2d(const rdeic_conv_desc* d, void* stream) { return conv2d_impl(d, -2, stream); }

extern "C" int rdeic_conv2d_tile(const rdeic_conv_desc* d, int32_t tile, void* stream) {
  return conv2d_impl(d, tile, stream);
}

extern "C" int rdeic_conv2d_splitk(const rdeic_conv_desc* d, int32_t splits, float* ws, size_t ws_floats,
                                   void* stream) {
  if (d && d->gn_part && (d->gn_hw <= 0 || d->gn_hw % 64 || (long)d->n * d->ho * d->wo % d->gn_hw))
    return RDEIC_EINVAL;
  int rc;
  {
    rdeic_prof_add_bytes(conv_bytes(d));
    ProfScope ps((hipStream_t)stream, RDEIC_PROF_CONV, conv_flops(d));
    rc = conv2d_splitk_impl(d, splits, ws, ws_floats, stream);
  }
  if (rc == RDEIC_OK) rdeic_count_launch(RDEIC_COUNT_SPLITK);
  if (rc != RDEIC_OK || !d->gn_part) return rc;
  return gn_rows_partial(d->out, (long)d->n * d->ho * d->wo, d->cout, d->out_ld, d->gn_hw, d->gn_part,
                         d->out_f32 ? 0 : 1, (hipStream_t)stream);
}

extern "C" int rdeic_set_conv_path(int32_t path) {
  int prev = g_conv_path;
  g_conv_path = path;
  return prev;
}

extern int rdeic_g_attn64;
extern int rdeic_g_attn512;

extern "C" int rdeic_set_conv_option(int32_t key, int32_t value) {
  if (key == 0) { int prev = g_epi_vec; g_epi_vec = value; return prev; }
  if (key == 1) { int prev = rdeic_g_attn64; rdeic_g_attn64 = value; return prev; }
  if (key == 3) { int prev = g_swz; g_swz = value; return prev; }
  if (key == 4) { int prev = g_force_tile; g_force_tile = value; return prev; }
  if (key == 5) { int prev = g_dma; g_dma = value; return prev; }
  if (key == 6) { int prev = g_halo; g_halo = value; return prev; }
  if (key == 8) { int prev = rdeic_g_attn512; rdeic_g_attn512 = value; return prev; }
  if (key == 9) { int prev = g_halo8; g_halo8 = value; return prev; }
  if (key == 10) { int prev = g_edge; g_edge = value; return prev; }
  return RDEIC_EINVAL;
}
```

rdeic_amd/ops.py:

```python
from __future__ import annotations

import ctypes as C
import json
import math
import os
import threading
from dataclasses import dataclass
from typing import Optional

import torch

from . import _lib
from ._lib import ConvDesc, call

NONE, LEAKY, GELU, SILU = 0, 1, 2, 3


def dt_code(t: torch.Tensor) -> int:
    if t.dtype == torch.bfloat16:
        return 1
    if t.dtype == torch.float32:
        return 0
    raise TypeError(f"unsupported activation dtype {t.dtype}")


def stream_ptr() -> int:
    return torch.cuda.current_stream().cuda_stream


def _ptr(t: Optional[torch.Tensor]) -> Optional[int]:
    return None if t is None else t.data_ptr()


def pix_ld(x: torch.Tensor) -> int:
    if x.dim() != 4 or x.stride(3) != 1:
        raise ValueError(f"expected NHWC activation with contiguous channels, got shape {tuple(x.shape)} "
                         f"strides {x.stride()}")
    n, h, w, c = x.shape
    ld = x.stride(2)
    if ld < c or (h > 1 and x.stride(1) != w * ld) or (n > 1 and x.stride(0) != h * w * ld):
        raise ValueError(f"activation pixels not evenly strided: shape {tuple(x.shape)} strides {x.stride()}")
    return ld


def new_act(n: int, h: int, w: int, c: int, dtype, device=None) -> torch.Tensor:
    return torch.empty((n, h, w, c), dtype=dtype, device=device or "cuda")


@dataclass
class ConvParams:
    weight: torch.Tensor
    wld: int
    bias: Optional[torch.Tensor]
    cout: int
    cin: int
    kh: int
    kw: int
    stride: int = 1
    pad: int = 0
    ln_cs: Optional[torch.Tensor] = None

    @staticmethod
    def pack(w: torch.Tensor, b: Optional[torch.Tensor], stride: int = 1, pad: int = 0,
             dtype=torch.bfloat16) -> "ConvParams":
        if w.dim() == 2:
            w = w[:, :, None, None]
        w = w.detach().to(device="cuda", dtype=torch.float32).contiguous()
        cout, cin, kh, kw = w.shape
        wld = ((kh * kw * cin + 63) // 64) * 64
        packed = torch.empty((cout, wld), dtype=dtype, device="cuda")
        call("rdeic_pack_conv_weight", w.data_ptr(), cout, cin, kh, kw, packed.data_ptr(), wld,
             1 if dtype == torch.bfloat16 else 0, stream_ptr())
        bias = None if b is None else b.detach().to(device="cuda", dtype=torch.float32).contiguous()
        return ConvParams(packed, wld, bias, cout, cin, kh, kw, stride, pad)


def conv2d(x: torch.Tensor, p: ConvParams, *, x2: Optional[torch.Tensor] = None, up2: bool = False,
           pad_t: Optional[int] = None, pad_l: Optional[int] = None, out_hw=None,
           gn: Optional[torch.Tensor] = None, gn_silu: bool = False, emb: Optional[torch.Tensor] = None,
           act: int = NONE, slope: float = 0.0, res: Optional[torch.Tensor] = None,
           out: Optional[torch.Tensor] = None, out_f32: bool = False, pixel_shuffle: bool = False,
           geglu: bool = False, stats: bool = False, stats_hw: Optional[int] = None,
           images: Optional[int] = None, ln_rows: Optional[torch.Tensor] = None) -> torch.Tensor:
    if gn is not None and _gn_materialize(x, x2, p) and not _halo_eligible(x, x2, p, up2, pad_t, pad_l, out_hw,
                                                                           geglu or pixel_shuffle, out) \
            and not _edge_narrow_eligible(x, x2, p, up2, pad_t, pad_l, out_hw, geglu or pixel_shuffle or emb is not None):
        xin = torch.empty(x.shape[:3] + (p.cin,), dtype=x.dtype, device=x.device)
        c0 = x.shape[3]
        pend = getattr(gn, "_rdeic_pending", None)
        if pend is not None and c0 % 8 == 0 and pix_ld(x) % 8 == 0 and x.data_ptr() % 16 == 0 and \
                (x2 is None or (x2.shape[3] % 8 == 0 and pix_ld(x2) % 8 == 0 and x2.data_ptr() % 16 == 0)):
            p0, pc0, p1, c1, n_, hw_, groups, eps, gamma, beta = pend
            _launch(("gn_apply", float(2 * xin.numel() * xin.element_size()), None), "rdeic_groupnorm_parts_apply",
                    p0.data_ptr(), pc0, _ptr(p1), c1, x.data_ptr(), pix_ld(x), _ptr(x2),
                    pix_ld(x2) if x2 is not None else 0, n_, hw_, groups, float(eps), gamma.data_ptr(),
                    beta.data_ptr(), int(gn_silu), gn.data_ptr(), xin.data_ptr(), pix_ld(xin), stream_ptr())
            del gn._rdeic_pending
        else:
            group_norm_apply(x, gn, gn_silu, out=xin[..., :c0])
            if x2 is not None:
                group_norm_apply(x2, gn[:, c0:], gn_silu, out=xin[..., c0:])
        x, x2, gn = xin, None, None
    n, h, w, c0 = x.shape
    ld0 = pix_ld(x)
    c1, ld1 = 0, 0
    if x2 is not None:
        if x2.shape[:3] != x.shape[:3] or x2.dtype != x.dtype:
            raise ValueError("concat inputs must share n, h, w and dtype")
        c1 = x2.shape[3]
        ld1 = pix_ld(x2)
    if c0 + c1 != p.cin:
        raise ValueError(f"conv expects cin={p.cin}, got {c0}+{c1}")
    if p.weight.dtype != x.dtype:
        raise TypeError(f"weight dtype {p.weight.dtype} != activation dtype {x.dtype}")
    hi, wi = (2 * h, 2 * w) if up2 else (h, w)
    pt = p.pad if pad_t is None else pad_t
    pl = p.pad if pad_l is None else pad_l
    if out_hw is None:
        ho = (hi + 2 * p.pad - p.kh) // p.stride + 1
        wo = (wi + 2 * p.pad - p.kw) // p.stride + 1
    else:
        ho, wo = out_hw
    odt = torch.float32 if (out_f32 or x.dtype == torch.float32) else x.dtype
    if geglu:
        if x.dtype != torch.bfloat16 or c0 % 64 or c1 % 64 or p.cout % 8 or res is not None or emb is not None \
                or act != NONE or out_f32 or pixel_shuffle:
            raise ValueError("fused GEGLU: bf16, 64-channel-aligned input, no residual / emb / activation")
        oshape = (n, ho, wo, p.cout // 2)
    elif pixel_shuffle:
        oshape = (n, 2 * ho, 2 * wo, p.cout // 4)
    else:
        oshape = (n, ho, wo, p.cout)
    if out is None:
        out = torch.empty(oshape, dtype=odt, device=x.device)
    elif tuple(out.shape) != oshape or out.dtype != odt:
        raise ValueError(f"out has shape {tuple(out.shape)}/{out.dtype}, expected {oshape}/{odt}")
    d = ConvDesc()
    d.in0 = x.data_ptr()
    d.in1 = _ptr(x2)
    d.c0, d.c1, d.ld0, d.ld1 = c0, c1, ld0, ld1
    d.n, d.h, d.w, d.up2 = n, h, w, int(up2)
    d.weight, d.wld, d.bias = p.weight.data_ptr(), p.wld, _ptr(p.bias)
    d.cout, d.kh, d.kw, d.stride, d.pad_t, d.pad_l = p.cout, p.kh, p.kw, p.stride, pt, pl
    d.ho, d.wo = ho, wo
    if gn is not None:
        if gn.shape != (n, p.cin, 2):
            raise ValueError("gn affine must be [n, cin, 2]")
        _ab_ready(gn)
        d.gn_ab = gn.data_ptr()
        d.gn_silu = int(gn_silu)
    if emb is not None:
        if emb.dtype != torch.float32 or emb.shape[0] != n or emb.stride(1) != 1:
            raise ValueError("emb must be fp32 [n, >=cout] row-major")
        d.emb = emb.data_ptr()
        d.emb_ld = emb.stride(0)
    d.act, d.act_param = act, float(slope)
    if res is not None:
        if tuple(res.shape) != oshape or res.dtype != odt:
            raise ValueError(f"residual {tuple(res.shape)}/{res.dtype} does not match output {oshape}/{odt}")
        d.res = res.data_ptr()
        d.res_ld = pix_ld(res)
    d.out = out.data_ptr()
    d.out_ld = pix_ld(out)
    d.out_mode = 2 if geglu else (1 if pixel_shuffle else 0)
    d.dtype = dt_code(x)
    d.out_f32 = int(odt == torch.float32 and x.dtype != torch.float32)
    d.batch = 1
    if ln_rows is not None:
        if p.ln_cs is None or ln_rows.dtype != torch.float32 or tuple(ln_rows.shape) != (n * ho * wo, 2) \
                or not ln_rows.is_contiguous():
            raise ValueError("ln_rows needs a ParamStore.conv_ln weight and an fp32 [M, 2] contiguous (mean, rstd)")
        d.ln_rows, d.ln_colsum = ln_rows.data_ptr(), p.ln_cs.data_ptr()
    elif p.ln_cs is not None:
        raise ValueError("a LayerNorm-folded weight needs ln_rows")
    part = None
    if stats and GN_STATS_FUSE and x.dtype == torch.bfloat16 and not (geglu or pixel_shuffle):
        ghw = int(stats_hw or ho * wo)
        nf = int(_lib.load().rdeic_groupnorm_parts_floats(n * ho * wo, p.cout, ghw))
        if nf:
            part = torch.empty(nf, dtype=torch.float32, device=x.device)
            d.gn_part, d.gn_hw = part.data_ptr(), ghw
    flops = 2.0 * n * ho * wo * p.cout * p.kh * p.kw * p.cin
    splits = _splitk_count(x, x2, n * ho * wo, p, gn is not None or pixel_shuffle or geglu, out,
                           n if images is None else images)

    tile = -1
    if splits == 1 and x.dtype == torch.bfloat16 and gn is None and _gn_materialize(x, x2, p):
        key = tile_key(n * ho * wo, c0, c1, p, up2, d.out_mode, res is not None, emb is not None, act, odt)
        tile = TILE_TABLE.get(key, -1) if FORCE_TILE is None else FORCE_TILE
        if AUTOTUNE and FORCE_TILE is None and key not in TILE_TABLE:
            scratch = torch.empty_strided(out.size(), out.stride(), dtype=out.dtype, device=out.device)
            dma = c0 % 64 == 0 and c1 % 64 == 0
            tile = _autotune_tile(d, scratch, DMA_TILE_CANDIDATES if dma else TILE_CANDIDATES)
            if tile >= 0:
                TILE_TABLE[key] = tile

    tag = ("conv", flops, (n, h, w, c0, c1, p.cout, p.kh, p.stride, gn is not None, int(up2), d.out_mode))
    if splits > 1:
        ws = _splitk_workspace(splits * n * ho * wo * p.cout, x.device)
        _launch(tag, "rdeic_conv2d_splitk", C.byref(d), splits, ws.data_ptr(), ws.numel(), stream_ptr())
    elif tile >= 0:
        _launch(tag, "rdeic_conv2d_tile", C.byref(d), tile, stream_ptr())
    else:
        _launch(tag, "rdeic_conv2d", C.byref(d), stream_ptr())
    if part is not None:
        _attach_gn_part(out, part, d.gn_hw)
    return out


GN_STATS_FUSE = True


def _attach_gn_part(t: torch.Tensor, part: torch.Tensor, hw: int) -> None:
    t._rdeic_gn_part = (part, t.data_ptr(), tuple(t.shape), tuple(t.stride()), hw)


def _gn_part_of(t: Optional[torch.Tensor], hw: int):
    info = getattr(t, "_rdeic_gn_part", None) if t is not None else None
    if info is None:
        return None
    part, ptr, shape, stride, phw = info
    if ptr != t.data_ptr() or shape != tuple(t.shape) or stride != tuple(t.stride()) or phw != hw:
        return None
    return part


AUTOTUNE = False
FORCE_TILE: Optional[int] = None
GEGLU_FUSED = True
TILE_CANDIDATES = (0, 1, 3, 4, 6, 8, 10)
DMA_TILE_CANDIDATES = (25, 32, 34, 26, 30, 33, 24, 31, 35, 36, 37, 38)
ALL_TILES = (0, 1, 2, 3, 4, 6, 7, 8, 9, 10) + tuple(range(21, 39))
TILE_TABLE_PATH = os.environ.get("RDEIC_TILE_TABLE") or os.path.join(os.path.dirname(os.path.abspath(__file__)),
                                                                     "conv_tiles.json")


def tile_key(m: int, c0: int, c1: int, p: "ConvParams", up2: bool, out_mode: int, res: bool, emb: bool, act: int,
             odt) -> str:
    return (f"m{m}:c{c0}+{c1}:o{p.cout}:k{p.kh}x{p.kw}:s{p.stride}:up{int(up2)}:om{out_mode}:"
            f"r{int(res)}:e{int(emb)}:a{act}:{'f32' if odt == torch.float32 else 'bf16'}")


def _load_tile_table() -> dict:
    if not os.path.exists(TILE_TABLE_PATH):
        return {}
    with open(TILE_TABLE_PATH) as f:
        tab = json.load(f)["tiles"]
    bad = {k: v for k, v in tab.items() if v not in ALL_TILES}
    if bad:
        raise ValueError(f"{TILE_TABLE_PATH}: unknown tile ids {bad}")
    return tab


TILE_TABLE: dict = _load_tile_table()


def _autotune_tile(d0, scratch: torch.Tensor, candidates=None) -> int:
    if _lib.RECORDER is not None:
        return -1
    d = ConvDesc.from_buffer_copy(d0)
    d.out = scratch.data_ptr()
    s = stream_ptr()
    best, best_t = -1, float("inf")
    for t in (TILE_CANDIDATES if candidates is None else candidates):
        call("rdeic_conv2d_tile", C.byref(d), t, s)
        e0 = torch.cuda.Event(enable_timing=True)
        e1 = torch.cuda.Event(enable_timing=True)
        e0.record()
        for _ in range(2):
            call("rdeic_conv2d_tile", C.byref(d), t, s)
        e1.record()
        e1.synchronize()
        ms = e0.elapsed_time(e1)
        if ms < best_t:
            best, best_t = t, ms
    return best


_SPLITK_WS: dict = {}
_SPLITK_TLS = threading.local()


def splitk_state():
    return getattr(_SPLITK_TLS, "allowed", False), getattr(_SPLITK_TLS, "short", False)


SPLITK_NOMINAL_BATCH = 16
SPLITK_BLOCKS, SPLITK_MAX = 512, 8
SPLITK_TRAIN = None
SPLITK_ENTROPY = True


class splitk_allowed:

    def __init__(self, short_k: bool = False):
        self.short_k = short_k

    def __enter__(self):
        self._prev = splitk_state()
        _SPLITK_TLS.allowed, _SPLITK_TLS.short = True, self.short_k or self._prev[1]
        return self

    def __exit__(self, *exc):
        _SPLITK_TLS.allowed, _SPLITK_TLS.short = self._prev


class splitk_as:

    def __init__(self, state):
        self.state = tuple(state)

    def __enter__(self):
        self._prev = splitk_state()
        _SPLITK_TLS.allowed, _SPLITK_TLS.short = self.state
        return self

    def __exit__(self, *exc):
        _SPLITK_TLS.allowed, _SPLITK_TLS.short = self._prev


def _splitk_count(x, x2, M: int, p: "ConvParams", fused: bool, out: torch.Tensor, n: int) -> int:
    allowed, short = splitk_state()
    if not short:
        M = (M // max(1, n)) * SPLITK_NOMINAL_BATCH
    if not allowed or fused or x.dtype not in (torch.bfloat16, torch.float32) or p.cout % 8 \
            or pix_ld(out) % 8 or out.data_ptr() % 16:
        return 1
    for t in (x, x2):
        if t is not None and (t.shape[3] % 8 or pix_ld(t) % 8 or t.data_ptr() % 16):
            return 1
    if x.dtype == torch.float32:
        tiles = -(-M // 64) * -(-p.cout // 64)
        nk = -(-(p.kh * p.kw * p.cin) // 32)
        if short and tiles < 256 and 8 <= nk < 32:
            return max(1, min(-(-512 // tiles), nk // 4, 16))
        if tiles >= 256 or nk < 32:
            return 1
        return max(1, min(-(-512 // tiles), nk // 8, 16))
    tiles = -(-M // 128) * -(-p.cout // 128)
    nk = -(-(p.kh * p.kw * p.cin) // 64)
    if short and tiles < 128 and 8 <= nk < 32:
        return max(1, min(-(-512 // tiles), nk // 4, 8))
    if short and SPLITK_TRAIN is not None and tiles < 192 and nk >= 32:
        kdiv, smax, target = SPLITK_TRAIN
        return max(1, min(-(-target // tiles), nk // kdiv, smax))
    if tiles >= 192 or nk < 32:
        return 1
    return max(1, min(SPLITK_BLOCKS // tiles, nk // 16, SPLITK_MAX))


_SPLITK_KEEP: list = []


def _splitk_workspace(n: int, device) -> torch.Tensor:
    key = (str(device), stream_ptr())
    buf = _SPLITK_WS.get(key)
    if buf is None or buf.numel() < n:
        buf = torch.empty(n, dtype=torch.float32, device=device)
        _SPLITK_WS[key] = buf
        _SPLITK_KEEP.append(buf)
    return buf


PROFILE = None
PROFILE_OTHER: dict = {}


def _launch(tag, name: str, *args):
    if PROFILE is None:
        return call(name, *args, tag=tag)
    ev0 = torch.cuda.Event(enable_timing=True)
    ev1 = torch.cuda.Event(enable_timing=True)
    ev0.record()
    call(name, *args, tag=tag)
    ev1.record()
    record_profile(tag, ev0, ev1)


def record_profile(tag, ev0, ev1):
    kind, work, meta = tag
    if kind == "conv":
        PROFILE.append((work, ev0, ev1, None, meta))
    else:
        PROFILE_OTHER.setdefault(kind, []).append((work, ev0, ev1))


PROF_KINDS = {"conv": 0, "attention": 1, "attention_dh16": 2, "gn_stats": 3, "gn_apply": 4, "gemm": 5,
              "attention_d512": 6, "conv_bytes": 7}


def prof_start(capacity: int = 65536, every: int = 1) -> None:
    call("rdeic_prof_start", capacity, every)


def prof_stop() -> int:
    return int(_lib.load().rdeic_prof_stop())


def prof_read() -> dict:
    out = {}
    for kind, code in PROF_KINDS.items():
        n, w, ms = C.c_int64(), C.c_double(), C.c_double()
        call("rdeic_prof_read", code, C.byref(n), C.byref(w), C.byref(ms))
        if n.value:
            out[kind] = (n.value, w.value, ms.value)
    return out


def prof_read_keys(kind: str, cap: int = 64) -> list:
    keys, n = (C.c_int64 * cap)(), (C.c_int64 * cap)()
    w, ms = (C.c_double * cap)(), (C.c_double * cap)()
    m = int(_lib.load().rdeic_prof_read_keys(PROF_KINDS[kind], keys, n, w, ms, cap))
    return [(int(keys[i]), int(n[i]), float(w[i]), float(ms[i])) for i in range(max(0, m))]


def attention_key(key: int) -> dict:
    return {"dh": (key >> 48) & 0xffff, "lq": (key >> 32) & 0xffff, "lk": (key >> 16) & 0xffff, "bh": key & 0xffff}


def other_profile_summary():
    out = {}
    for kind, recs in PROFILE_OTHER.items():
        out[kind] = (len(recs), sum(r[0] for r in recs), sum(r[1].elapsed_time(r[2]) for r in recs))
    return out


def conv_profile_summary(records):
    total_ms = 0.0
    total_flops = 0.0
    for rec in records:
        flops, e0, e1 = rec[0], rec[1], rec[2]
        total_ms += e0.elapsed_time(e1)
        total_flops += flops
    return len(records), total_flops, total_ms


def conv_profile_breakdown(records):
    out = {}
    for rec in records:
        flops, e0, e1, meta = rec[0], rec[1], rec[2], rec[4]
        key = str(meta)
        v = out.setdefault(key, [0, 0.0, 0.0])
        v[0] += 1
        v[1] += flops / 1e9
        v[2] += e0.elapsed_time(e1)
    return out


CONV_PATH = 2


def set_conv_path(path: int) -> int:
    global CONV_PATH
    prev = CONV_PATH
    CONV_PATH = int(path)
    _lib.load().rdeic_set_conv_path(CONV_PATH)
    return prev


def set_conv_option(key: int, value: int) -> int:
    return int(_lib.load().rdeic_set_conv_option(int(key), int(value)))


HALO_CONV = 1
HALO_MAX_C = 512


COUNT_HALO_CONV, COUNT_GN_APPLY, COUNT_LAYERNORM, COUNT_HALO_SMALL, COUNT_LN_FUSED, COUNT_SPLITK, COUNT_EDGE, \
    COUNT_GN_PARTS_APPLY = 0, 1, 2, 3, 4, 5, 6, 7


def launch_count(kind: int) -> int:
    return int(_lib.load().rdeic_launch_count(int(kind)))


def launch_count_reset() -> None:
    call("rdeic_launch_count_reset")


def set_halo_conv(mode: int) -> int:
    global HALO_CONV
    prev = HALO_CONV
    HALO_CONV = int(mode)
    _lib.load().rdeic_set_conv_option(6, HALO_CONV)
    return prev


def _halo_eligible(x, x2, p: "ConvParams", up2, pad_t, pad_l, out_hw, special, out) -> bool:
    if not HALO_CONV or x.dtype != torch.bfloat16 or x2 is not None or up2 or special:
        return False
    if p.kh != 3 or p.kw != 3 or p.stride != 1 or p.pad != 1 or (pad_t not in (None, 1)) or (pad_l not in (None, 1)):
        return False
    n, h, w, c = x.shape
    if out_hw is not None and tuple(out_hw) != (h, w):
        return False
    if c % 32 or c > min(512, HALO_MAX_C) or p.cout > HALO_MAX_C or p.cout % 128 or h % 4 or w % 64 \
            or x.stride(2) % 8 or x.data_ptr() % 16:
        return False
    if out is not None and (pix_ld(out) % 8 or out.data_ptr() % 16):
        return False
    return True


EDGE_CONV = 1


def set_edge_conv(mode: int) -> int:
    global EDGE_CONV
    prev = EDGE_CONV
    EDGE_CONV = int(mode)
    _lib.load().rdeic_set_conv_option(10, EDGE_CONV)
    return prev


def _edge_narrow_eligible(x, x2, p: "ConvParams", up2, pad_t, pad_l, out_hw, special) -> bool:
    if not EDGE_CONV or x.dtype != torch.bfloat16 or x2 is not None or up2 or special:
        return False
    if p.kh != 3 or p.kw != 3 or p.stride != 1 or p.pad != 1 or (pad_t not in (None, 1)) or (pad_l not in (None, 1)):
        return False
    n, h, w, c = x.shape
    if out_hw is not None and tuple(out_hw) != (h, w):
        return False
    lds = 10 * 66 * 64 + c * 8 + p.cout * 9 * c * 2
    return p.cout <= 16 and c % 32 == 0 and lds <= 160 * 1024 and h % 8 == 0 and w % 64 == 0 \
        and x.stride(2) % 8 == 0 and x.data_ptr() % 16 == 0


def _gn_materialize(x: torch.Tensor, x2: Optional[torch.Tensor], p: ConvParams) -> bool:
    if CONV_PATH == 0 or x.dtype != torch.bfloat16:
        return False
    if p.cout <= 32 and not (p.cout <= 4 and x.shape[0] * x.shape[1] * x.shape[2] >= (1 << 20)):
        return False
    for t in (x, x2):
        if t is None:
            continue
        if t.shape[3] % 8 or t.stride(2) % 8 or t.data_ptr() % 16:
            return False
    return True


def linear(x: torch.Tensor, p: ConvParams, *, act: int = NONE, res: Optional[torch.Tensor] = None,
           out: Optional[torch.Tensor] = None, out_f32: bool = False, geglu: bool = False,
           stats_hw: Optional[int] = None, images: int, ln_rows: Optional[torch.Tensor] = None) -> torch.Tensor:
    rows, c = x.shape
    x4 = x.as_strided((1, rows, 1, c), (rows * x.stride(0), x.stride(0), x.stride(0), 1))
    odt = torch.float32 if (out_f32 or x.dtype == torch.float32) else x.dtype
    cw = p.cout // 2 if geglu else p.cout
    if out is None:
        out = torch.empty((rows, cw), dtype=odt, device=x.device)
    o4 = out.as_strided((1, rows, 1, cw), (rows * out.stride(0), out.stride(0), out.stride(0), 1))
    r4 = None
    if res is not None:
        r4 = res.as_strided((1, rows, 1, p.cout), (rows * res.stride(0), res.stride(0), res.stride(0), 1))
    conv2d(x4, p, act=act, res=r4, out=o4, out_f32=out_f32, geglu=geglu, stats=stats_hw is not None,
           stats_hw=stats_hw, images=images, ln_rows=ln_rows)
    info = getattr(o4, "_rdeic_gn_part", None)
    if info is not None:
        out._rdeic_gn_tokens = info
    return out


def tokens_to_nhwc(t: torch.Tensor, n: int, h: int, w: int) -> torch.Tensor:
    v = t.view(n, h, w, t.shape[1])
    info = getattr(t, "_rdeic_gn_tokens", None)
    if info is not None and info[4] == h * w:
        _attach_gn_part(v, info[0], h * w)
    return v


def gemm_batched(a: torch.Tensor, b_nk: torch.Tensor, out: torch.Tensor, *, batch: int, m: int, n: int, k: int,
                 lda: int, ldb: int, a_bs: int, b_bs: int, out_bs: int) -> torch.Tensor:
    d = ConvDesc()
    d.in0 = a.data_ptr()
    d.c0, d.ld0 = k, lda
    d.n, d.h, d.w = 1, m, 1
    d.weight, d.wld = b_nk.data_ptr(), ldb
    d.cout, d.kh, d.kw, d.stride = n, 1, 1, 1
    d.ho, d.wo = m, 1
    d.out = out.data_ptr()
    d.out_ld = n
    d.dtype = dt_code(a)
    d.out_f32 = int(out.dtype == torch.float32 and a.dtype != torch.float32)
    d.batch = batch
    d.in_bs, d.w_bs, d.out_bs = a_bs, b_bs, out_bs
    _launch(("conv", 2.0 * batch * m * n * k, ("bgemm", batch, m, n, k)), "rdeic_conv2d", C.byref(d), stream_ptr())
    return out


GN_PARTS_APPLY = True
GN_PARTS_APPLY_HW = (64, 128, 256)


def _ab_ready(ab: Optional[torch.Tensor]) -> None:
    pend = getattr(ab, "_rdeic_pending", None) if ab is not None else None
    if pend is None:
        return
    p0, c0, p1, c1, n, hw, groups, eps, gamma, beta = pend
    call("rdeic_groupnorm_parts_ab", p0.data_ptr(), c0, _ptr(p1), c1, n, hw, groups, float(eps),
         gamma.data_ptr(), beta.data_ptr(), ab.data_ptr(), stream_ptr())
    del ab._rdeic_pending


def group_norm_ab(x: torch.Tensor, gamma: torch.Tensor, beta: torch.Tensor, groups: int, eps: float,
                  x2: Optional[torch.Tensor] = None, defer: bool = False) -> torch.Tensor:
    n, h, w, c0 = x.shape
    ld0 = pix_ld(x)
    c1, ld1 = (x2.shape[3], pix_ld(x2)) if x2 is not None else (0, 0)
    c = c0 + c1
    p0, p1 = _gn_part_of(x, h * w), _gn_part_of(x2, h * w)
    if p0 is not None and (x2 is None or p1 is not None):
        ab = torch.empty((n, c, 2), dtype=torch.float32, device=x.device)
        if defer and GN_PARTS_APPLY and h * w in GN_PARTS_APPLY_HW and x.dtype == torch.bfloat16 and groups <= 256:
            ab._rdeic_pending = (p0, c0, p1, c1, n, h * w, groups, float(eps), gamma, beta)
            return ab
        call("rdeic_groupnorm_parts_ab", p0.data_ptr(), c0, _ptr(p1), c1, n, h * w, groups, float(eps),
             gamma.data_ptr(), beta.data_ptr(), ab.data_ptr(), stream_ptr())
        return ab
    ws = torch.empty(int(_lib.load().rdeic_groupnorm_ws_floats(n, h * w, c)), dtype=torch.float32, device=x.device)
    ab = torch.empty((n, c, 2), dtype=torch.float32, device=x.device)
    _launch(("gn_stats", float(n * h * w * c * x.element_size()), None),
            "rdeic_groupnorm_stats", x.data_ptr(), c0, ld0, _ptr(x2), c1, ld1, n, h * w, groups,
            float(eps), gamma.data_ptr(), beta.data_ptr(), ab.data_ptr(), ws.data_ptr(), dt_code(x), stream_ptr())
# ... 138 lines not shown
```

rdeic_amd/params.py:

```python
from __future__ import annotations

from typing import Dict, Iterable, Optional, Sequence, Tuple

import torch

from . import ops
from . import weights as W


class ParamStore:
    def __init__(self, compute_dtype=torch.bfloat16, device="cuda"):
        self.compute_dtype = compute_dtype
        self.device = torch.device(device)
        self.shapes: Dict[str, Tuple[int, ...]] = {}
        self.t: Dict[str, torch.Tensor] = {}
        self._packed: Dict[tuple, ops.ConvParams] = {}

    def declare(self, name: str, shape: Sequence[int]):
        shape = tuple(int(s) for s in shape)
        if name in self.shapes and self.shapes[name] != shape:
            raise ValueError(f"{name} declared twice with different shapes")
        self.shapes[name] = shape

    def declare_conv(self, prefix: str, cout: int, cin: int, k: int, bias: bool = True):
        self.declare(prefix + ".weight", (cout, cin, k, k))
        if bias:
            self.declare(prefix + ".bias", (cout,))

    def declare_linear(self, prefix: str, cout: int, cin: int, bias: bool = True):
        self.declare(prefix + ".weight", (cout, cin))
        if bias:
            self.declare(prefix + ".bias", (cout,))

    def declare_norm(self, prefix: str, c: int):
        self.declare(prefix + ".weight", (c,))
        self.declare(prefix + ".bias", (c,))

    def init_synthetic(self, global_seed: int = W.GLOBAL_SEED, rate_gain: float = 1.0):
        for name, shape in self.shapes.items():
            scale, offset = W.init_spec(name, shape, rate_gain)
            t = torch.empty(shape, dtype=torch.float32, device=self.device)
            ops.fill_uniform(t, W.param_seed(name, global_seed), scale, offset)
            self.t[name] = t
        self._packed.clear()

    def load_state_dict(self, sd: Dict[str, torch.Tensor], strict: bool = True):
        missing = [n for n in self.shapes if n not in sd]
        if strict and missing:
            raise KeyError(f"missing parameters: {missing[:8]}{' ...' if len(missing) > 8 else ''}")
        for name, shape in self.shapes.items():
            if name not in sd:
                continue
            v = sd[name]
            if tuple(v.shape) != shape:
                raise ValueError(f"{name}: checkpoint shape {tuple(v.shape)} != {shape}")
            self.t[name] = v.detach().to(device=self.device, dtype=torch.float32).contiguous()
        self._packed.clear()

    def names(self) -> Iterable[str]:
        return self.shapes.keys()

    def get(self, name: str) -> torch.Tensor:
        return self.t[name]

    def has(self, name: str) -> bool:
        return name in self.shapes

    def conv(self, prefix: str, stride: int = 1, pad: Optional[int] = None, dtype=None,
             scale: float = 1.0, cin_pad: Optional[int] = None, cout_pad: Optional[int] = None) -> ops.ConvParams:
        dtype = dtype or self.compute_dtype
        key = (prefix, stride, pad, dtype, scale, cin_pad, cout_pad)
        p = self._packed.get(key)
        if p is None:
            w = self.t[prefix + ".weight"]
            b = self.t.get(prefix + ".bias")
            if scale != 1.0:
                w, b = w * scale, (None if b is None else b * scale)
            if cin_pad is not None and cin_pad > w.shape[1]:
                w = torch.nn.functional.pad(w, (0, 0) * (w.dim() - 2) + (0, cin_pad - w.shape[1]))
            if cout_pad is not None and cout_pad > w.shape[0]:
                w = torch.nn.functional.pad(w, (0, 0) * (w.dim() - 1) + (0, cout_pad - w.shape[0]))
                if b is not None:
                    b = torch.nn.functional.pad(b, (0, cout_pad - b.shape[0]))
            k = w.shape[-1] if w.dim() == 4 else 1
            p = ops.ConvParams.pack(w, b, stride=stride, pad=(k // 2 if pad is None else pad), dtype=dtype)
            self._packed[key] = p
        return p

    def conv_split_pad(self, prefix: str, c0: int, c0_pad: int, dtype=None) -> ops.ConvParams:
        dtype = dtype or self.compute_dtype
        key = (prefix, "split_pad", c0, c0_pad, dtype)
        p = self._packed.get(key)
        if p is None:
            w = self.t[prefix + ".weight"]
            cout, cin, kh, kw = w.shape
            wp = torch.zeros((cout, cin - c0 + c0_pad, kh, kw), dtype=w.dtype, device=w.device)
            wp[:, :c0] = w[:, :c0]
            wp[:, c0_pad:] = w[:, c0:]
            p = ops.ConvParams.pack(wp, self.t.get(prefix + ".bias"), stride=1, pad=kh // 2, dtype=dtype)
            self._packed[key] = p
        return p

    def conv_geglu(self, prefix: str, dtype=None) -> ops.ConvParams:
        dtype = dtype or self.compute_dtype
        key = (prefix, "geglu", dtype)
        p = self._packed.get(key)
        if p is None:
            w = self.t[prefix + ".weight"]
            b = self.t.get(prefix + ".bias")
            c = w.shape[0] // 2
            if c % 4:
                raise ValueError("GEGLU width must be a multiple of 4")
            perm = torch.arange(2 * c, device=w.device).view(2, c // 4, 4).permute(1, 0, 2).reshape(-1)
            p = ops.ConvParams.pack(w[perm], None if b is None else b[perm], dtype=dtype)
            self._packed[key] = p
        return p

    def conv_ln(self, prefixes: Sequence[str], ln_prefix: str, geglu: bool = False, dtype=None) -> ops.ConvParams:
        dtype = dtype or self.compute_dtype
        key = (tuple(prefixes), "ln", ln_prefix, geglu, dtype)
        p = self._packed.get(key)
        if p is None:
            gamma, beta = self.t[ln_prefix + ".weight"], self.t[ln_prefix + ".bias"]
            ws, bs = [], []
            for pre in prefixes:
                w = self.t[pre + ".weight"]
                b = self.t.get(pre + ".bias")
                ws.append(w)
                bs.append(b if b is not None else torch.zeros(w.shape[0], device=self.device))
            w = torch.cat(ws, 0)
            b = torch.cat(bs, 0).double() + w.double() @ beta.double()
            w = w * gamma[None, :]
            if geglu:
                c = w.shape[0] // 2
                perm = torch.arange(2 * c, device=w.device).view(2, c // 4, 4).permute(1, 0, 2).reshape(-1)
                w, b = w[perm], b[perm]
            p = ops.ConvParams.pack(w, b.float(), dtype=dtype)
            p.ln_cs = p.weight.double().sum(1).float().contiguous()
            self._packed[key] = p
        return p

    def conv_cat(self, prefixes: Sequence[str], dtype=None) -> ops.ConvParams:
        dtype = dtype or self.compute_dtype
        key = (tuple(prefixes), "cat", dtype)
        p = self._packed.get(key)
        if p is None:
            ws, bs = [], []
            for pre in prefixes:
                w = self.t[pre + ".weight"]
                ws.append(w if w.dim() == 4 else w[:, :, None, None])
                b = self.t.get(pre + ".bias")
                bs.append(b if b is not None else torch.zeros(w.shape[0], device=self.device))
            any_bias = any(self.t.get(pre + ".bias") is not None for pre in prefixes)
            w = torch.cat(ws, 0)
            p = ops.ConvParams.pack(w, torch.cat(bs, 0) if any_bias else None, stride=1, pad=w.shape[-1] // 2,
                                    dtype=dtype)
            self._packed[key] = p
        return p
```

rdeic_amd/unet.py:

```python
from __future__ import annotations

from dataclasses import dataclass, field
from typing import List, Optional

import torch

from . import ops
from .params import ParamStore


def find_denominator(number: int, start: int) -> int:
    if start >= number:
        return number
    while start != 0:
        if number % start == 0:
            return start
        start -= 1
    return 1


@dataclass
class ResBlock:
    prefix: str
    cin: int
# ... 78 lines not shown
                store.declare_linear(f"{tb}.{a}.to_q", inner, ch, bias=False)
                store.declare_linear(f"{tb}.{a}.to_k", inner, kv_in, bias=False)
                store.declare_linear(f"{tb}.{a}.to_v", inner, kv_in, bias=False)
                store.declare_linear(f"{tb}.{a}.to_out.0", ch, inner)
            store.declare_linear(tb + ".ff.net.0.proj", inner * 8, inner)
            store.declare_linear(tb + ".ff.net.2", inner, inner * 4)
            for nn_ in ("norm1", "norm2", "norm3"):
                store.declare_norm(f"{tb}.{nn_}", inner)
            store.declare_linear(pre + ".proj_out", inner, ch)
            return SpatialTransformer(pre, ch, heads, dh, find_denominator(ch, 32))

        nhc_cur = nhc
        self.input_blocks: List[list] = []
        p0 = prefix + "input_blocks.0.0"
        store.declare_conv(p0, mc, in_ch, 3)
        self.input_blocks.append([Conv(p0, in_ch, mc)])
        chans, ch, ds, idx = [mc], mc, 1, 1
        for level, mult in enumerate(mults):
            for _ in range(nrb):
                layers = [res(f"{prefix}input_blocks.{idx}.0", ch, mult * mc)]
                ch = mult * mc
                if ds in attn_res:
                    layers.append(st(f"{prefix}input_blocks.{idx}.1", ch))
                self.input_blocks.append(layers)
                chans.append(ch)
                idx += 1
            if level != len(mults) - 1:
                pre = f"{prefix}input_blocks.{idx}.0.op"
                store.declare_conv(pre, ch, ch, 3)
                self.input_blocks.append([Down(pre, ch)])
                chans.append(ch)
                ds *= 2
                idx += 1
        self.enc_out_ch = list(chans)
        self.middle = [res(prefix + "middle_block.0", ch, ch), st(prefix + "middle_block.1", ch),
                       res(prefix + "middle_block.2", ch, ch)]
        self.mid_ch = ch
        self.output_blocks: List[list] = []
        self.dec_out_ch: List[int] = []
        if not control:
            k = 0
            for level, mult in list(enumerate(mults))[::-1]:
                for i in range(nrb + 1):
                    ich = chans.pop()
                    layers = [res(f"{prefix}output_blocks.{k}.0", ch + ich, mc * mult)]
                    ch = mc * mult
                    if ds in attn_res:
                        layers.append(st(f"{prefix}output_blocks.{k}.1", ch))
                    if level and i == nrb:
                        pre = f"{prefix}output_blocks.{k}.{len(layers)}.conv"
                        store.declare_conv(pre, ch, ch, 3)
                        layers.append(Up(pre, ch))
                        ds //= 2
                    self.output_blocks.append(layers)
                    self.dec_out_ch.append(ch)
                    k += 1
            store.declare_norm(prefix + "out.0", ch)
            store.declare_conv(prefix + "out.2", cfg["out_channels"], mc, 3)
        off = 0
        for rb in self.resblocks:
            rb.emb_off = off
            off += rb.cout
        self.emb_total = off

    def time_embed(self, temb: torch.Tensor) -> torch.Tensor:
        s = self.store
        B = temb.shape[0]
        e = ops.linear(temb, s.conv(self.prefix + "time_embed.0", dtype=torch.float32), act=ops.SILU, images=B)
        e = ops.linear(e, s.conv(self.prefix + "time_embed.2", dtype=torch.float32), act=ops.SILU, images=B)
        stacked = s.conv_cat([rb.prefix + ".emb_layers.1" for rb in self.resblocks], dtype=torch.float32)
        return ops.linear(e, stacked, images=B)

    def resblock(self, rb: ResBlock, x: torch.Tensor, emb_all: torch.Tensor,
                 x2: Optional[torch.Tensor] = None, stats: bool = False) -> torch.Tensor:
        s = self.store
        ab1 = ops.group_norm_ab(x, s.get(rb.prefix + ".in_layers.0.weight"), s.get(rb.prefix + ".in_layers.0.bias"),
                                rb.gn_in, 1e-5, x2=x2, defer=True)
        h = ops.conv2d(x, s.conv(rb.prefix + ".in_layers.2"), x2=x2, gn=ab1, gn_silu=True,
                       emb=emb_all[:, rb.emb_off:rb.emb_off + rb.cout], stats=True)
        ab2 = ops.group_norm_ab(h, s.get(rb.prefix + ".out_layers.0.weight"),
                                s.get(rb.prefix + ".out_layers.0.bias"), rb.gn_out, 1e-5, defer=True)
        if rb.cin != rb.cout:
            skip = ops.conv2d(x, s.conv(rb.prefix + ".skip_connection"), x2=x2)
        else:
            if x2 is not None:
                raise ValueError("identity skip with a concatenated input")
            skip = x
        return ops.conv2d(h, s.conv(rb.prefix + ".out_layers.3"), gn=ab2, gn_silu=True, res=skip, stats=stats)

    def transformer(self, t: SpatialTransformer, x: torch.Tensor, ctx_kv_in: torch.Tensor, ctx_batch: int,
                    ctx_len: int, stats: bool = False) -> torch.Tensor:
        s = self.store
        B, H, W_, C = x.shape
        L = H * W_
        rows = B * L
        tb = t.prefix + ".transformer_blocks.0"
        ab = ops.group_norm_ab(x, s.get(t.prefix + ".norm.weight"), s.get(t.prefix + ".norm.bias"), t.gn, 1e-6,
                               defer=True)
        h4 = ops.conv2d(x, s.conv(t.prefix + ".proj_in"), gn=ab, gn_silu=False)
        h = h4.view(rows, C)
        scale = t.dh ** -0.5
        fold = x.dtype == torch.bfloat16 and ops.LN_FOLD and C % 64 == 0
        qkv_names = [tb + ".attn1.to_q", tb + ".attn1.to_k", tb + ".attn1.to_v"]
        if fold:
            qkv = ops.linear(h, s.conv_ln(qkv_names, tb + ".norm1"), ln_rows=ops.layer_norm_rowstats(h), images=B)
        else:
            n1 = ops.layer_norm(h, s.get(tb + ".norm1.weight"), s.get(tb + ".norm1.bias"))
            qkv = ops.linear(n1, s.conv_cat(qkv_names), images=B)
        o = torch.empty((rows, C), dtype=x.dtype, device=x.device)
        ops.attention(qkv[:, :C], qkv[:, C:2 * C], qkv[:, 2 * C:], o, batch=B, heads=t.heads, lq=L, lk=L, dh=t.dh,
                      scale=scale)
        h = ops.linear(o, s.conv(tb + ".attn1.to_out.0"), res=h, images=B)
        if fold:
            q = ops.linear(h, s.conv_ln([tb + ".attn2.to_q"], tb + ".norm2"), ln_rows=ops.layer_norm_rowstats(h),
                           images=B)
        else:
            n2 = ops.layer_norm(h, s.get(tb + ".norm2.weight"), s.get(tb + ".norm2.bias"))
            q = ops.linear(n2, s.conv(tb + ".attn2.to_q"), images=B)
        kv = ops.linear(ctx_kv_in, s.conv_cat([tb + ".attn2.to_k", tb + ".attn2.to_v"]), images=ctx_batch)
        ops.attention(q, kv[:, :C], kv[:, C:], o, batch=B, heads=t.heads, lq=L, lk=ctx_len, dh=t.dh, scale=scale,
                      kv_bcast=(ctx_batch == 1 and B > 1))
        h = ops.linear(o, s.conv(tb + ".attn2.to_out.0"), res=h, images=B)
        if fold and ops.GEGLU_FUSED:
            gg = ops.linear(h, s.conv_ln([tb + ".ff.net.0.proj"], tb + ".norm3", geglu=True),
                            ln_rows=ops.layer_norm_rowstats(h), geglu=True, images=B)
        else:
            n3 = ops.layer_norm(h, s.get(tb + ".norm3.weight"), s.get(tb + ".norm3.bias"))
            if x.dtype == torch.bfloat16 and ops.GEGLU_FUSED and C % 64 == 0:
                gg = ops.linear(n3, s.conv_geglu(tb + ".ff.net.0.proj"), geglu=True, images=B)
            else:
                gg = ops.geglu(ops.linear(n3, s.conv(tb + ".ff.net.0.proj"), images=B))
        h = ops.linear(gg, s.conv(tb + ".ff.net.2"), res=h, images=B)
        if not x.is_contiguous():
            raise ValueError("transformer input must be contiguous NHWC")
        out = ops.linear(h, s.conv(t.prefix + ".proj_out"), res=x.view(rows, C), stats_hw=L if stats else None,
                         images=B)
        return ops.tokens_to_nhwc(out, B, H, W_)

    def run_layers(self, layers, x, emb_all, ctx_rows, ctx_batch, ctx_len, x2=None, stats_last: bool = True):
        s = self.store
        for li, layer in enumerate(layers):
            st = stats_last or li + 1 < len(layers)
            if isinstance(layer, Conv):
                x = ops.conv2d(x, s.conv(layer.prefix), x2=x2, stats=st)
                x2 = None
            elif isinstance(layer, ResBlock):
                x = self.resblock(layer, x, emb_all, x2=x2, stats=st)
                x2 = None
            elif isinstance(layer, SpatialTransformer):
                x = self.transformer(layer, x, ctx_rows, ctx_batch, ctx_len, stats=st)
            elif isinstance(layer, Down):
                x = ops.conv2d(x, s.conv(layer.prefix, stride=2, pad=1), stats=st)
            elif isinstance(layer, Up):
                x = ops.conv2d(x, s.conv(layer.prefix), up2=True, stats=st)
            else:
                raise TypeError(layer)
        return x


class NoiseEstimator:

    def __init__(self, store: ParamStore, unet_cfg: dict, control_cfg: dict,
                 base_prefix: str = "model.diffusion_model.", ctrl_prefix: str = "control_model."):
        self.store = store
        self.base = UNet(store, base_prefix, unet_cfg, control=False)
        self.ctrl = UNet(store, ctrl_prefix + "control_model.", control_cfg, control=True)
        self.model_channels = unet_cfg["model_channels"]
        self.control_scale = float(control_cfg.get("control_scale", 1.0))
        cp = ctrl_prefix
        enc_c, enc_b = self.ctrl.enc_out_ch, self.base.enc_out_ch
        self.enc_zero = [f"{cp}enc_zero_convs_out.{i}.0" for i in range(len(enc_c))]
        for i, pre in enumerate(self.enc_zero):
            store.declare_conv(pre, enc_b[i], enc_c[i], 1)
        self.mid_zero = f"{cp}middle_block_out.0"
        store.declare_conv(self.mid_zero, self.base.mid_ch, self.ctrl.mid_ch, 1)
        self.dec_zero = []
        for i in range(len(enc_c)):
            pre = f"{cp}dec_zero_convs_out.{i}.0"
            cout = self.base.mid_ch if i == 0 else self.base.dec_out_ch[i - 1]
            store.declare_conv(pre, cout, enc_c[-(i + 1)], 1)
            self.dec_zero.append(pre)
        half = self.model_channels // 2
        import math
        self._freqs_cpu = torch.exp(-math.log(10000) * torch.arange(start=0, end=half, dtype=torch.float32) / half)
        self._freqs = None

    def _pad64(self, x: torch.Tensor) -> torch.Tensor:
        B, H, W_, c = x.shape
        key = (B, H, W_, x.dtype, ops.stream_ptr())
        cache = self.__dict__.setdefault("_pad_cache", {})
        buf = cache.get(key)
        if buf is None:
            buf = torch.zeros((B, H, W_, 64), dtype=x.dtype, device=x.device)
            cache[key] = buf
        xc = x.contiguous()
        ops.call("rdeic_act_fwd", xc.data_ptr(), B * H * W_, c, c, None, 0, 0, 0.0, buf.data_ptr(), 64,
                 ops.dt_code(x), ops.stream_ptr())
        return buf

    def timestep_embedding(self, t: torch.Tensor) -> torch.Tensor:
        if self._freqs is None:
            self._freqs = self._freqs_cpu.to(t.device)
        B = t.shape[0]
        out = torch.empty((B, self.model_channels), dtype=torch.float32, device=t.device)
        ops.call("rdeic_timestep_embedding", t.data_ptr(), self._freqs.data_ptr(), B, self.model_channels,
                 out.data_ptr(), ops.stream_ptr())
        return out

    def forward(self, x: torch.Tensor, hint: torch.Tensor, t: torch.Tensor, ctx: torch.Tensor) -> torch.Tensor:
        with ops.splitk_allowed():
            return self._forward(x, hint, t, ctx)

    def forward_unconditional(self, x: torch.Tensor, t: torch.Tensor, ctx: torch.Tensor) -> torch.Tensor:
        with ops.splitk_allowed():
            s = self.store
            dt = s.compute_dtype
            t = t.to(device=x.device, dtype=torch.int64).contiguous()
            emb_b = self.base.time_embed(self.timestep_embedding(t))
            ctx = ctx.to(dt).contiguous()
            Bc, Lc, Dc = ctx.shape
            ctx_rows = ctx.view(Bc * Lc, Dc)
            h_base = ops.cast(x, dt)
            hs_base = []
            for lb in self.base.input_blocks:
                h_base = self.base.run_layers(lb, h_base, emb_b, ctx_rows, Bc, Lc)
                hs_base.append(h_base)
            h_base = self.base.run_layers(self.base.middle, h_base, emb_b, ctx_rows, Bc, Lc)
            for lb in self.base.output_blocks:
                h_base = self.base.run_layers(lb, h_base, emb_b, ctx_rows, Bc, Lc, x2=hs_base.pop())
            p = self.base.prefix
            ab = ops.group_norm_ab(h_base, s.get(p + "out.0.weight"), s.get(p + "out.0.bias"), 32, 1e-5)
            return ops.conv2d(h_base, s.conv(p + "out.2"), gn=ab, gn_silu=True, out_f32=True)

    def _forward(self, x: torch.Tensor, hint: torch.Tensor, t: torch.Tensor, ctx: torch.Tensor) -> torch.Tensor:
        s = self.store
        dt = s.compute_dtype
        B = x.shape[0]
        t = t.to(device=x.device, dtype=torch.int64).contiguous()
        temb = self.timestep_embedding(t)
        emb_c = self.ctrl.time_embed(temb)
        emb_b = self.base.time_embed(temb)
        ctx = ctx.to(dt).contiguous()
        Bc, Lc, Dc = ctx.shape
        ctx_rows = ctx.view(Bc * Lc, Dc)
        sc = self.control_scale * self.control_scale
        h_base = ops.cast(x, dt)
        h_ctr, ctr_x2 = h_base, hint
        hs_base, hs_ctr = [], []
        for i, (lb, lc) in enumerate(zip(self.base.input_blocks, self.ctrl.input_blocks)):
            h_base0 = h_base
            h_base = self.base.run_layers(lb, h_base, emb_b, ctx_rows, Bc, Lc, stats_last=False)
            if i == 0 and dt == torch.bfloat16 and len(lc) == 1 and isinstance(lc[0], Conv) and \
                    h_base0.shape[3] % 64 and hint.shape[3] % 64 == 0:
                h_ctr = ops.conv2d(self._pad64(h_base0), s.conv_split_pad(lc[0].prefix, h_base0.shape[3], 64),
                                   x2=hint, stats=True)
            else:
                h_ctr = self.ctrl.run_layers(lc, h_ctr, emb_c, ctx_rows, Bc, Lc, x2=ctr_x2)
            ctr_x2 = None
            h_base = ops.conv2d(h_ctr, s.conv(self.enc_zero[i], scale=sc), res=h_base, stats=True)
            hs_base.append(h_base)
            hs_ctr.append(h_ctr)
        h_base = self.base.run_layers(self.base.middle, h_base, emb_b, ctx_rows, Bc, Lc, stats_last=False)
        h_ctr = self.ctrl.run_layers(self.ctrl.middle, h_ctr, emb_c, ctx_rows, Bc, Lc, stats_last=False)
        h_base = ops.conv2d(h_ctr, s.conv(self.mid_zero, scale=sc), res=h_base, stats=True)
        nout = len(self.base.output_blocks)
        for i, lb in enumerate(self.base.output_blocks):
            h_base = ops.conv2d(hs_ctr.pop(), s.conv(self.dec_zero[i], scale=sc), res=h_base, stats=True)
            h_base = self.base.run_layers(lb, h_base, emb_b, ctx_rows, Bc, Lc, x2=hs_base.pop(),
                                          stats_last=(i + 1 == nout))
        p = self.base.prefix
        ab = ops.group_norm_ab(h_base, s.get(p + "out.0.weight"), s.get(p + "out.0.bias"), 32, 1e-5)
        return ops.conv2d(h_base, s.conv(p + "out.2"), gn=ab, gn_silu=True, out_f32=True)
```

rdeic_amd/vae.py:

```python
from __future__ import annotations

import torch

from . import ops
from .params import ParamStore

GN_EPS = 1e-6


class AutoencoderKL:
    def __init__(self, store: ParamStore, dd: dict, embed_dim: int, prefix: str = "first_stage_model."):
        self.store, self.prefix, self.dd = store, prefix, dd
        ch, chm, nrb = dd["ch"], dd["ch_mult"], dd["num_res_blocks"]
        zc = dd["z_channels"]
        self.nres = len(chm)
        e = prefix + "encoder."
        store.declare_conv(e + "conv_in", ch, dd["in_channels"], 3)
        in_chm = (1,) + tuple(chm)
        self.enc_blocks = []
        block_in = ch
        for i in range(self.nres):
            block_in = ch * in_chm[i]
            block_out = ch * chm[i]
            lvl = []
            for j in range(nrb):
                lvl.append(self._declare_resnet(f"{e}down.{i}.block.{j}", block_in, block_out))
                block_in = block_out
            down = None
            if i != self.nres - 1:
                down = f"{e}down.{i}.downsample.conv"
                store.declare_conv(down, block_in, block_in, 3)
            self.enc_blocks.append((lvl, down))
        self.enc_mid = (self._declare_resnet(e + "mid.block_1", block_in, block_in),
                        self._declare_attn(e + "mid.attn_1", block_in),
                        self._declare_resnet(e + "mid.block_2", block_in, block_in))
        store.declare_norm(e + "norm_out", block_in)
        store.declare_conv(e + "conv_out", 2 * zc if dd["double_z"] else zc, block_in, 3)
        self.enc_out_ch = block_in
        store.declare_conv(prefix + "quant_conv", 2 * embed_dim, 2 * zc, 1)
        store.declare_conv(prefix + "post_quant_conv", zc, embed_dim, 1)
        d = prefix + "decoder."
        block_in = ch * chm[-1]
        store.declare_conv(d + "conv_in", block_in, zc, 3)
        self.dec_mid = (self._declare_resnet(d + "mid.block_1", block_in, block_in),
                        self._declare_attn(d + "mid.attn_1", block_in),
                        self._declare_resnet(d + "mid.block_2", block_in, block_in))
        self.dec_blocks = []
        for i in reversed(range(self.nres)):
            block_out = ch * chm[i]
            lvl = []
            for j in range(nrb + 1):
                lvl.append(self._declare_resnet(f"{d}up.{i}.block.{j}", block_in, block_out))
                block_in = block_out
            up = None
            if i != 0:
                up = f"{d}up.{i}.upsample.conv"
                store.declare_conv(up, block_in, block_in, 3)
            self.dec_blocks.append((lvl, up))
        store.declare_norm(d + "norm_out", block_in)
        store.declare_conv(d + "conv_out", dd["out_ch"], block_in, 3)

    def _declare_resnet(self, pre, cin, cout):
        s = self.store
        s.declare_norm(pre + ".norm1", cin)
        s.declare_conv(pre + ".conv1", cout, cin, 3)
        s.declare_norm(pre + ".norm2", cout)
        s.declare_conv(pre + ".conv2", cout, cout, 3)
        if cin != cout:
            s.declare_conv(pre + ".nin_shortcut", cout, cin, 1)
        return (pre, cin, cout)

    def _declare_attn(self, pre, c):
        s = self.store
        s.declare_norm(pre + ".norm", c)
        for n in ("q", "k", "v", "proj_out"):
            s.declare_conv(f"{pre}.{n}", c, c, 1)
        return (pre, c)

    def resnet(self, blk, x):
        pre, cin, cout = blk
        s = self.store
        ab1 = ops.group_norm_ab(x, s.get(pre + ".norm1.weight"), s.get(pre + ".norm1.bias"), 32, GN_EPS)
        h = ops.conv2d(x, s.conv(pre + ".conv1"), gn=ab1, gn_silu=True, stats=True)
        ab2 = ops.group_norm_ab(h, s.get(pre + ".norm2.weight"), s.get(pre + ".norm2.bias"), 32, GN_EPS)
        skip = x if cin == cout else ops.conv2d(x, s.conv(pre + ".nin_shortcut"))
        return ops.conv2d(h, s.conv(pre + ".conv2"), gn=ab2, gn_silu=True, res=skip, stats=True)

    def attn(self, blk, x):
        pre, c = blk
        s = self.store
        B, H, W_, C = x.shape
        L = H * W_
        ab = ops.group_norm_ab(x, s.get(pre + ".norm.weight"), s.get(pre + ".norm.bias"), 32, GN_EPS)
        qkv = ops.conv2d(x, s.conv_cat([pre + ".q", pre + ".k", pre + ".v"]), gn=ab, gn_silu=False)
        qkv = qkv.view(B * L, 3 * C)
        o = torch.empty((B * L, C), dtype=x.dtype, device=x.device)
        if x.dtype == torch.bfloat16 and C == 512 and L % 32 == 0 and ops.VAE_FLASH_ATTENTION:
            ops.attention(qkv[:, :C], qkv[:, C:2 * C], qkv[:, 2 * C:], o, batch=B, heads=1, lq=L, lk=L, dh=C,
                          scale=int(C) ** (-0.5))
        else:
            ops.attention_single_head_materialized(qkv[:, :C], qkv[:, C:2 * C], qkv[:, 2 * C:], o, batch=B,
                                                   length=L, dim=C, scale=int(C) ** (-0.5))
        out = ops.linear(o, s.conv(pre + ".proj_out"), res=x.contiguous().view(B * L, C), stats_hw=L,
                          images=B)
        return ops.tokens_to_nhwc(out, B, H, W_)

    def encode_hc(self, x: torch.Tensor, out_mul: float = 1.0) -> torch.Tensor:
        return self._encode(x, out_mul, moments=False)

    def encode_hc_moments(self, x: torch.Tensor, out_mul: float = 1.0):
        return self._encode(x, out_mul, moments=True)

    def _encode(self, x: torch.Tensor, out_mul: float, moments: bool):
        s = self.store
        e = self.prefix + "encoder."
        h = ops.conv2d(x, s.conv(e + "conv_in", cin_pad=x.shape[3] if x.shape[3] > 3 else None), stats=True)
        for lvl, down in self.enc_blocks:
            for blk in lvl:
                h = self.resnet(blk, h)
            if down is not None:
                Hh, Ww = h.shape[1], h.shape[2]
                h = ops.conv2d(h, s.conv(down, stride=2, pad=0), pad_t=0, pad_l=0, out_hw=(Hh // 2, Ww // 2),
                               stats=True)
        h = self.resnet(self.enc_mid[0], h)
        h = self.attn(self.enc_mid[1], h)
        h = self.resnet(self.enc_mid[2], h)
        ab = ops.group_norm_ab(h, s.get(e + "norm_out.weight"), s.get(e + "norm_out.bias"), 32, GN_EPS)
        if not moments:
            return ops.group_norm_apply(h, ab, silu=True, out_mul=out_mul)
        c = ops.group_norm_apply(h, ab, silu=True)
        hc = ops.conv2d(c, s.conv(e + "conv_out"), out_f32=True)
        mom = ops.conv2d(hc, s.conv(self.prefix + "quant_conv", dtype=torch.float32))
        if out_mul != 1.0:
            c = ops.group_norm_apply(h, ab, silu=True, out_mul=out_mul)
        return c, mom

    def decode(self, z: torch.Tensor, out_f32: bool = True) -> torch.Tensor:
        s = self.store
        d = self.prefix + "decoder."
        z = ops.conv2d(z, s.conv(self.prefix + "post_quant_conv"))
        h = ops.conv2d(z, s.conv(d + "conv_in"), stats=True)
        h = self.resnet(self.dec_mid[0], h)
        h = self.attn(self.dec_mid[1], h)
        h = self.resnet(self.dec_mid[2], h)
        for lvl, up in self.dec_blocks:
            for blk in lvl:
                h = self.resnet(blk, h)
            if up is not None:
                h = ops.conv2d(h, s.conv(up), up2=True, stats=True)
        ab = ops.group_norm_ab(h, s.get(d + "norm_out.weight"), s.get(d + "norm_out.bias"), 32, GN_EPS)
        return ops.conv2d(h, s.conv(d + "conv_out"), gn=ab, gn_silu=True, out_f32=out_f32)
```

Baseline: 152.0 images/s.

## Fold nearest-upsample plus 3x3 conv into four 2x2 phase convolutions

Replaces the nearest-neighbour 2x upsample followed by a 3x3 conv with four 2x2 sub-pixel phase convolutions over the low-resolution input, using weights pre-folded on the host once per layer. Each output phase is written through a pixel-mapping epilogue, and GroupNorm partial stats are remapped to the right slots. This removes the redundant MACs (9 taps per output drop to 4) and the reads of the upsampled input, in the VAE decoder and UNet up blocks. The cost is a new kernel variant, extra folded weight memory, and bf16 rounding of the folded weights, which can differ slightly from the original conv.

Measured after the change: 159.8 images/s, median of 6. +5.1%, better.

```diff
diff --git a/include/rdeic_hip.h b/include/rdeic_hip.h
--- a/include/rdeic_hip.h
+++ b/include/rdeic_hip.h
@@ -46,6 +46,8 @@
 int rdeic_conv2d(const rdeic_conv_desc* d, void* stream);
 int rdeic_conv2d_tile(const rdeic_conv_desc* d, int32_t tile, void* stream);
 int rdeic_conv2d_splitk(const rdeic_conv_desc* d, int32_t splits, float* ws, size_t ws_floats, void* stream);
+int rdeic_conv2d_up2_phases(const rdeic_conv_desc* d, int64_t phase_stride, int32_t tile, void* stream);
+int rdeic_conv2d_up2_group(const rdeic_conv_desc* d);
 int rdeic_set_conv_path(int32_t path);
 int rdeic_set_conv_option(int32_t key, int32_t value);
 
diff --git a/rdeic_amd/_lib.py b/rdeic_amd/_lib.py
--- a/rdeic_amd/_lib.py
+++ b/rdeic_amd/_lib.py
@@ -63,6 +63,8 @@
     "rdeic_conv2d": (C.c_int, [C.POINTER(ConvDesc), _p]),
     "rdeic_conv2d_splitk": (C.c_int, [C.POINTER(ConvDesc), _i32, _p, C.c_size_t, _p]),
     "rdeic_conv2d_tile": (C.c_int, [C.POINTER(ConvDesc), _i32, _p]),
+    "rdeic_conv2d_up2_phases": (C.c_int, [C.POINTER(ConvDesc), _i64, _i32, _p]),
+    "rdeic_conv2d_up2_group": (C.c_int, [C.POINTER(ConvDesc)]),
     "rdeic_prof_start": (C.c_int, [_i32, _i32]),
     "rdeic_prof_stop": (C.c_int, []),
     "rdeic_launch_count": (C.c_int64, [_i32]),
@@ -206,3 +208,14 @@
         RECORDER.append((name, fn, args, tag))
     rc = fn(*args)
     check(name, rc)
+
+
+def call_soft(name: str, *args, tag=None) -> bool:
+    fn = getattr(load(), name)
+    rc = fn(*args)
+    if rc == 1:
+        return False
+    check(name, rc)
+    if RECORDER is not None:
+        RECORDER.append((name, fn, args, tag))
+    return True
diff --git a/rdeic_amd/csrc/coders.cpp b/rdeic_amd/csrc/coders.cpp
--- a/rdeic_amd/csrc/coders.cpp
+++ b/rdeic_amd/csrc/coders.cpp
@@ -420,7 +420,7 @@
 
 int rdeic_version(void) { return 1; }
 
-int rdeic_abi_count(void) { return 93; }
+int rdeic_abi_count(void) { return 95; }
 
 static int pmf_to_quantized_cdf_impl(const float* pmf, int32_t n, int32_t precision, uint32_t* cdf_out) {
   if (!pmf || !cdf_out || n <= 0 || precision <= 0 || precision > 24) return RDEIC_EINVAL;
diff --git a/rdeic_amd/csrc/conv_common.h b/rdeic_amd/csrc/conv_common.h
--- a/rdeic_amd/csrc/conv_common.h
+++ b/rdeic_amd/csrc/conv_common.h
@@ -93,10 +93,31 @@
   __device__ __forceinline__ int operator()(int r) const { return m0 + r; }
 };
 
-template <int BM, int BN, int WGM, int WGN, int NT, int P = 2, class RowMap = RowsFrom, bool PF = true>
+struct PixSame {
+  __device__ __forceinline__ long operator()(int m) const { return m; }
+  __device__ __forceinline__ long slot(int row0, int m) const { return (row0 + m) / 64; }
+};
+struct PixPhase {
+  int h, w, pa, pb;
+  __device__ __forceinline__ long operator()(int m) const {
+    const int hw = h * w;
+    const int img = m / hw, rem = m - img * hw;
+    const int i = rem / w, j = rem - i * w;
+    return ((long)img * (2 * h) + (2 * i + pa)) * (2 * w) + (2 * j + pb);
+  }
+  __device__ __forceinline__ long slot(int row0, int m) const {
+    const int b64 = (h * w) / 64;
+    const int r = (row0 + m) / 64;
+    const int img = r / b64, g = r - img * b64;
+    return (long)img * (4 * b64) + (2 * pa + pb) * b64 + g;
+  }
+};
+
+template <int BM, int BN, int WGM, int WGN, int NT, int P = 2, class RowMap = RowsFrom, bool PF = true,
+          class PixMap = PixSame>
 __device__ __forceinline__ void epilogue_vec(const f32x4 (&acc)[BM / WGM / 16][BN / WGN / 16], const ConvArgs& a,
                                              int m0, int n0, int wm, int wn, int lane, int tid, char* lds,
-                                             RowMap rmap = RowMap{0}) {
+                                             RowMap rmap = RowMap{0}, PixMap pmap = PixMap{}) {
   if constexpr (__is_same(RowMap, RowsFrom)) rmap.m0 = m0;
   constexpr int WTM = BM / WGM, WTN = BN / WGN;
   constexpr int TM = WTM / 16, TN = WTN / 16;
@@ -150,7 +171,7 @@
       lpf[k] = float2{0.f, 0.f};
       if (ok) {
         if (a.res && !of32 && a.out_mode != 2)
-          rpf[k] = *reinterpret_cast<const uint4*>(reinterpret_cast<const bf16*>(a.res) + (long)m * a.res_ld + nn);
+          rpf[k] = *reinterpret_cast<const uint4*>(reinterpret_cast<const bf16*>(a.res) + pmap(m) * a.res_ld + nn);
         if (a.ln_rows) lpf[k] = reinterpret_cast<const float2*>(a.ln_rows)[m];
       }
     }
@@ -230,20 +251,20 @@
       }
       if (a.res) {
         if (of32) {
-          const float4 r0 = *reinterpret_cast<const float4*>(reinterpret_cast<const float*>(a.res) + (long)m * a.res_ld + nn);
-          const float4 r1 = *reinterpret_cast<const float4*>(reinterpret_cast<const float*>(a.res) + (long)m * a.res_ld + nn + 4);
+          const float4 r0 = *reinterpret_cast<const float4*>(reinterpret_cast<const float*>(a.res) + pmap(m) * a.res_ld + nn);
+          const float4 r1 = *reinterpret_cast<const float4*>(reinterpret_cast<const float*>(a.res) + pmap(m) * a.res_ld + nn + 4);
           v[0] += r0.x; v[1] += r0.y; v[2] += r0.z; v[3] += r0.w; v[4] += r1.x; v[5] += r1.y; v[6] += r1.z; v[7] += r1.w;
         } else {
           bf16 rv[8];
           *reinterpret_cast<uint4*>(rv) =
               k < NPF ? rpf[k < NPF ? k : 0]
-                      : *reinterpret_cast<const uint4*>(reinterpret_cast<const bf16*>(a.res) + (long)m * a.res_ld + nn);
+                      : *reinterpret_cast<const uint4*>(reinterpret_cast<const bf16*>(a.res) + pmap(m) * a.res_ld + nn);
 #pragma unroll
           for (int e = 0; e < 8; ++e) v[e] += to_f32(rv[e]);
         }
       }
       if (of32) {
-        float* o = reinterpret_cast<float*>(a.out) + (long)m * a.out_ld + nn;
+        float* o = reinterpret_cast<float*>(a.out) + pmap(m) * a.out_ld + nn;
         *reinterpret_cast<float4*>(o) = make_float4(v[0], v[1], v[2], v[3]);
         *reinterpret_cast<float4*>(o + 4) = make_float4(v[4], v[5], v[6], v[7]);
         if (st) {
@@ -254,7 +275,7 @@
         bf16 ov[8];
 #pragma unroll
         for (int e = 0; e < 8; ++e) ov[e] = from_f32<bf16>(v[e]);
-        *reinterpret_cast<uint4*>(reinterpret_cast<bf16*>(a.out) + (long)m * a.out_ld + nn) = *reinterpret_cast<uint4*>(ov);
+        *reinterpret_cast<uint4*>(reinterpret_cast<bf16*>(a.out) + pmap(m) * a.out_ld + nn) = *reinterpret_cast<uint4*>(ov);
         if (st) {
           *reinterpret_cast<float4*>(L + pr * SDW + cc * 8) =
               make_float4(to_f32(ov[0]), to_f32(ov[1]), to_f32(ov[2]), to_f32(ov[3]));
@@ -305,7 +326,7 @@
         const int b = (tid + u * NT) / BN, j = (tid + u * NT) % BN;
         const int nn = n0 + j;
         if (b < BM / 64 && nn < a.cout && rmap(b * 64) < a.M) {
-          float* pp = a.gn_part + 4 + ((long)((a.gn_row0 + rmap(b * 64)) / 64) * a.cout + nn) * 2;
+          float* pp = a.gn_part + 4 + (pmap.slot(a.gn_row0, rmap(b * 64)) * a.cout + nn) * 2;
           pp[0] = ((sg[u][0] + sg[u][1]) + sg[u][2]) + sg[u][3];
           pp[1] = ((qg[u][0] + qg[u][1]) + qg[u][2]) + qg[u][3];
         }
@@ -470,7 +491,7 @@
   }
 }
 
-extern int g_conv_path, g_epi_vec, g_swz, g_force_tile, g_dma, g_halo, g_halo8, g_edge;
+extern int g_conv_path, g_epi_vec, g_swz, g_force_tile, g_dma, g_halo, g_halo8, g_edge, g_up2_phases;
 
 int make_args(const rdeic_conv_desc* d, ConvArgs& a, bool& vec);
 bool dma_ok(const rdeic_conv_desc* d, const ConvArgs& a, unsigned& b0, unsigned& b1, unsigned& bw);
@@ -480,4 +501,7 @@
 bool halo_ok(const rdeic_conv_desc* d, const ConvArgs& a);
 int launch_halo(const rdeic_conv_desc* d, ConvArgs a, hipStream_t s, bool* fused);
 int launch_edge(const rdeic_conv_desc* d, const ConvArgs& a, hipStream_t s, bool* fused);
-}
+int up2_phase_group(const rdeic_conv_desc* d);
+bool up2_phases_ok(const rdeic_conv_desc* d, long phase_stride);
+int launch_up2_phases(const rdeic_conv_desc* d, long phase_stride, int tile, hipStream_t s, bool* fused);
+}
diff --git a/rdeic_amd/csrc/conv_dma.hip b/rdeic_amd/csrc/conv_dma.hip
--- a/rdeic_amd/csrc/conv_dma.hip
+++ b/rdeic_amd/csrc/conv_dma.hip
@@ -2,9 +2,9 @@
 
 namespace rdeic_conv {
 
-template <int TM, int TN, int WTM, int WTN>
+template <int TM, int TN, int WTM, int WTN, class PixMap = PixSame>
 __device__ __forceinline__ void epilogue_scalar(const f32x4 (&acc)[TM][TN], const ConvArgs& a, int m0, int n0, int wm,
-                                                int wn, int lane) {
+                                                int wn, int lane, PixMap pmap = PixMap{}) {
   if (a.out_mode == 2) return;
   const int lrow = lane & 15, lq = lane >> 4;
   const int hw_o = a.ho * a.wo;
@@ -34,8 +34,8 @@
           oidx = p * a.out_ld + c;
           ridx = p * a.res_ld + c;
         } else {
-          oidx = (long)m * a.out_ld + nn;
-          ridx = (long)m * a.res_ld + nn;
+          oidx = pmap(m) * a.out_ld + nn;
+          ridx = pmap(m) * a.res_ld + nn;
         }
         if (a.res) v += of32 ? reinterpret_cast<const float*>(a.res)[ridx] : to_f32(reinterpret_cast<const bf16*>(a.res)[ridx]);
         if (of32) reinterpret_cast<float*>(a.out)[oidx] = v;
@@ -45,7 +45,7 @@
   }
 }
 
-template <int BM, int BN, int WGM, int WGN, int S, int EP, bool GEG = false>
+template <int BM, int BN, int WGM, int WGN, int S, int EP, bool GEG = false, bool PH = false>
 __device__ __forceinline__ void conv_dma_body(ConvArgs a, int tiles_n, unsigned bytes0, unsigned bytes1,
                                               unsigned bytesw) {
   constexpr int KB = 64;
@@ -65,6 +65,10 @@
   extern __shared__ __attribute__((aligned(16))) char lds[];
   HALO_STAMP(0);
 
+  if constexpr (PH) {
+    a.kh = 2; a.kw = 2; a.stride = 1; a.up2 = 0; a.c1 = 0; a.splits = 1;
+    a.res = nullptr; a.emb = nullptr; a.ln_rows = nullptr; a.out_f32 = 0; a.out_mode = 0;
+  }
   int kt_begin = 0, kt_end = a.nk;
   if (a.splits > 1) {
     const int z = blockIdx.z;
@@ -80,7 +84,16 @@
   const int nwg = gridDim.x, orig = blockIdx.x;
   const int xcd = orig & 7, q = nwg >> 3, rr = nwg & 7;
   const int wgid = (xcd < rr ? xcd * (q + 1) : rr * (q + 1) + (xcd - rr) * q) + (orig >> 3);
-  const int mt = wgid / tiles_n, nt = wgid - mt * tiles_n;
+  int mt = wgid / tiles_n;
+  const int nt = wgid - mt * tiles_n;
+  int phase = 0;
+  if constexpr (PH) {
+    phase = mt & 3;
+    mt >>= 2;
+    a.pad_t = 1 - (phase >> 1);
+    a.pad_l = 1 - (phase & 1);
+    a.weight += (long)phase * a.w_bs * 2;
+  }
   const int m0 = mt * BM, n0 = nt * BN;
 
   const int tid = threadIdx.x, lane = tid & 63;
@@ -208,6 +221,20 @@
   }
 
   HALO_STAMP(2);
+  if constexpr (PH) {
+    const PixPhase pm{a.h, a.w, phase >> 1, phase & 1};
+    if constexpr (TM % EP == 0 && (BM / EP) * (BN + 4) * 4 <= S * STAGE) {
+      if (a.epi_vec && epi_vec_ok(a)) {
+        epilogue_vec<BM, BN, WGM, WGN, NT, EP, RowsFrom, false, PixPhase>(acc, a, m0, n0, wm, wn, lane, tid, lds,
+                                                                          RowsFrom{m0}, pm);
+        HALO_STAMP(3);
+        return;
+      }
+    }
+    epilogue_scalar<TM, TN, WTM, WTN, PixPhase>(acc, a, m0, n0, wm, wn, lane, pm);
+    HALO_STAMP(3);
+    return;
+  }
   if constexpr (TM % EP == 0 && (BM / EP) * (BN + 4) * 4 <= S * STAGE) {
     if ((a.epi_vec || a.out_mode == 2) && epi_vec_ok(a)) {
       if constexpr (GEG) epilogue_geglu<BM, BN, WGM, WGN, NT, EP>(acc, a, m0, n0, wm, wn, lane, tid, lds);
@@ -220,10 +247,10 @@
   HALO_STAMP(3);
 }
 
-template <int BM, int BN, int WGM, int WGN, int S, int EP, bool GEG = false>
+template <int BM, int BN, int WGM, int WGN, int S, int EP, bool GEG = false, bool PH = false>
 __global__ __launch_bounds__(WGM * WGN * 64) void conv_dma_kernel(ConvArgs a, int tiles_n, unsigned bytes0,
                                                                   unsigned bytes1, unsigned bytesw) {
-  conv_dma_body<BM, BN, WGM, WGN, S, EP, GEG>(a, tiles_n, bytes0, bytes1, bytesw);
+  conv_dma_body<BM, BN, WGM, WGN, S, EP, GEG, PH>(a, tiles_n, bytes0, bytes1, bytesw);
 }
 
 template <int BM, int BN, int WGM, int WGN, int S, int EP, bool GEG = false>
@@ -350,4 +377,90 @@
   return RDEIC_OK;
 }
 
-}
+namespace {
+template <int BM, int BN, int WGM, int WGN, int S, int EP>
+int launch_dma_ph(ConvArgs a, unsigned b0, unsigned b1, unsigned bw, hipStream_t s, bool* fused) {
+  if (a.gn_part) {
+    const bool ok = (a.h * a.w) % 64 == 0 && stats_tile_ok<BM, BN, WGM, WGM * WGN * 64, EP>() &&
+                    dma_vec_epilogue<BM, BN, WGM, WGN, S, EP>(a);
+    if (!ok) a.gn_part = nullptr;
+    if (fused) *fused = ok;
+  }
+  const int tn = cdiv(a.cout, BN);
+  const long tiles = (long)cdiv(a.M, BM) * 4 * tn;
+  constexpr int lds = S * (BM + BN) * 128;
+  hipLaunchKernelGGL((conv_dma_kernel<BM, BN, WGM, WGN, S, EP, false, true>), dim3((unsigned)tiles),
+                     dim3(WGM * WGN * 64), lds, s, a, tn, b0, b1, bw);
+  return launch_status();
+}
+
+int launch_ph_auto(const ConvArgs& a, unsigned b0, unsigned b1, unsigned bw, hipStream_t s, int tile, bool* fused) {
+  if (tile != 32 && tile != 33 && tile != 25 && tile != 26 && tile != 30 && tile != 36) {
+    const long t128 = (long)cdiv(a.M, 128) * cdiv(a.cout, 128) * 4;
+    const long t256 = (long)cdiv(a.M, 256) * cdiv(a.cout, 256) * 4;
+    const float useful256 = (float)a.M * a.cout / ((float)cdiv(a.M, 256) * 256 * cdiv(a.cout, 256) * 256);
+    tile = (t256 >= 256 && useful256 >= 0.9f) ? 32 : t128 >= 256 ? 25 : 26;
+  }
+  switch (tile) {
+    case 32: return launch_dma_ph<256, 256, 4, 4, 2, 4>(a, b0, b1, bw, s, fused);
+    case 33: return launch_dma_ph<256, 128, 4, 4, 2, 2>(a, b0, b1, bw, s, fused);
+    case 25: return launch_dma_ph<128, 128, 2, 4, 2, 2>(a, b0, b1, bw, s, fused);
+    case 30: return launch_dma_ph<64, 128, 2, 2, 2, 2>(a, b0, b1, bw, s, fused);
+    case 36: return launch_dma_ph<64, 128, 2, 4, 2, 2>(a, b0, b1, bw, s, fused);
+    default: return launch_dma_ph<64, 128, 2, 2, 3, 2>(a, b0, b1, bw, s, fused);
+  }
+}
+}
+
+int up2_phase_group(const rdeic_conv_desc* d) {
+  const long ipix = (long)d->h * d->w;
+  const long per_in = ipix * d->ld0 * 2, per_out = 4 * ipix * d->out_ld * 2;
+  const long per = per_in > per_out ? per_in : per_out;
+  const long lim = (1l << 31) - 1;
+  if (d->n <= 0 || per <= 0 || per > lim) return 0;
+  long g = lim / per;
+  if (g > d->n) g = d->n;
+  const long groups = (d->n + g - 1) / g;
+  return (int)((d->n + groups - 1) / groups);
+}
+
+bool up2_phases_ok(const rdeic_conv_desc* d, long phase_stride) {
+  if (!d || !d->in0 || !d->weight || !d->out || d->n <= 0 || d->h <= 0 || d->w <= 0 || d->cout <= 0) return false;
+  if (d->dtype != 1 || d->out_f32 || !d->up2 || d->kh != 3 || d->kw != 3 || d->stride != 1 || d->pad_t != 1 ||
+      d->pad_l != 1 || d->ho != 2 * d->h || d->wo != 2 * d->w)
+    return false;
+  if (d->c1 || d->in1 || d->c0 <= 0 || d->c0 % 64 || d->out_mode != 0 || d->batch > 1) return false;
+  if (d->gn_ab || d->emb || d->res || d->ln_rows || d->ln_colsum) return false;
+  if (d->wld != 4 * d->c0 || phase_stride < (long)d->cout * d->wld || phase_stride % 8) return false;
+  if (d->ld0 < d->c0 || d->ld0 % 8 || ((uintptr_t)d->in0 % 16) || ((uintptr_t)d->weight % 16)) return false;
+  if (d->cout % 8 || d->out_ld < d->cout || d->out_ld % 8 || ((uintptr_t)d->out % 16)) return false;
+  if ((long)d->cout * d->wld * 2 >= (1l << 31)) return false;
+  return up2_phase_group(d) > 0;
+}
+
+int launch_up2_phases(const rdeic_conv_desc* d, long phase_stride, int tile, hipStream_t s, bool* fused) {
+  if (!up2_phases_ok(d, phase_stride)) return -1;
+  const int g = up2_phase_group(d);
+  const long ipix = (long)d->h * d->w;
+  const long per_in = ipix * d->ld0 * 2, per_out = 4 * ipix * d->out_ld * 2;
+  rdeic_conv_desc e = *d;
+  e.up2 = 0; e.kh = 2; e.kw = 2; e.stride = 1; e.pad_t = 1; e.pad_l = 1; e.ho = d->h; e.wo = d->w;
+  for (int i0 = 0; i0 < d->n; i0 += g) {
+    e.n = d->n - i0 < g ? d->n - i0 : g;
+    e.in0 = (const char*)d->in0 + i0 * per_in;
+    e.out = (char*)d->out + i0 * per_out;
+    ConvArgs ea;
+    bool vec = false;
+    unsigned b0, b1, bw;
+    if (make_args(&e, ea, vec) != RDEIC_OK || !vec || !dma_ok(&e, ea, b0, b1, bw)) return i0 == 0 ? -1 : RDEIC_EINVAL;
+    ea.w_bs = phase_stride;
+    ea.gn_row0 = (int)(i0 * ipix);
+    bool f = false;
+    const int rc = launch_ph_auto(ea, b0, b1, bw, s, tile, &f);
+    if (rc != RDEIC_OK) return rc;
+    if (fused) *fused = (i0 == 0 ? f : (*fused && f));
+  }
+  return RDEIC_OK;
+}
+
+}
diff --git a/rdeic_amd/csrc/conv_gemm.hip b/rdeic_amd/csrc/conv_gemm.hip
--- a/rdeic_amd/csrc/conv_gemm.hip
+++ b/rdeic_amd/csrc/conv_gemm.hip
@@ -9,6 +9,7 @@
 int g_dma = 1;
 int g_halo = 1;
 int g_halo8 = 1;
+int g_up2_phases = 1;
 
 namespace {
 
@@ -721,6 +722,27 @@
                          d->out_f32 ? 0 : 1, (hipStream_t)stream);
 }
 
+extern "C" int rdeic_conv2d_up2_phases(const rdeic_conv_desc* d, int64_t phase_stride, int32_t tile, void* stream) {
+  if (!d) return RDEIC_EINVAL;
+  if (!g_up2_phases || !g_dma || g_conv_path == 0) return 1;
+  if (d->gn_part && (d->gn_hw <= 0 || d->gn_hw % 64 || (long)d->n * d->ho * d->wo % d->gn_hw)) return RDEIC_EINVAL;
+  if (!up2_phases_ok(d, phase_stride)) return 1;
+  bool fused = false;
+  int rc;
+  {
+    const double pix = (double)d->n * d->h * d->w;
+    rdeic_prof_add_bytes(2.0 * (pix * d->c0 + 4.0 * d->cout * d->wld + 4.0 * pix * d->cout));
+    ProfScope ps((hipStream_t)stream, RDEIC_PROF_CONV, 2.0 * pix * 4.0 * d->c0 * d->cout * 4.0);
+    rc = launch_up2_phases(d, phase_stride, tile, (hipStream_t)stream, &fused);
+  }
+  if (rc == -1) return RDEIC_EINVAL;
+  if (rc != RDEIC_OK || !d->gn_part || fused) return rc;
+  return gn_rows_partial(d->out, (long)d->n * d->ho * d->wo, d->cout, d->out_ld, d->gn_hw, d->gn_part, 1,
+                         (hipStream_t)stream);
+}
+
+extern "C" int rdeic_conv2d_up2_group(const rdeic_conv_desc* d) { return d ? up2_phase_group(d) : 0; }
+
 extern "C" int rdeic_set_conv_path(int32_t path) {
   int prev = g_conv_path;
   g_conv_path = path;
@@ -740,5 +762,6 @@
   if (key == 8) { int prev = rdeic_g_attn512; rdeic_g_attn512 = value; return prev; }
   if (key == 9) { int prev = g_halo8; g_halo8 = value; return prev; }
   if (key == 10) { int prev = g_edge; g_edge = value; return prev; }
+  if (key == 11) { int prev = g_up2_phases; g_up2_phases = value; return prev; }
   return RDEIC_EINVAL;
 }
diff --git a/rdeic_amd/ops.py b/rdeic_amd/ops.py
--- a/rdeic_amd/ops.py
+++ b/rdeic_amd/ops.py
@@ -81,7 +81,8 @@
            act: int = NONE, slope: float = 0.0, res: Optional[torch.Tensor] = None,
            out: Optional[torch.Tensor] = None, out_f32: bool = False, pixel_shuffle: bool = False,
            geglu: bool = False, stats: bool = False, stats_hw: Optional[int] = None,
-           images: Optional[int] = None, ln_rows: Optional[torch.Tensor] = None) -> torch.Tensor:
+           images: Optional[int] = None, ln_rows: Optional[torch.Tensor] = None,
+           phases: Optional[ConvParams] = None) -> torch.Tensor:
     if gn is not None and _gn_materialize(x, x2, p) and not _halo_eligible(x, x2, p, up2, pad_t, pad_l, out_hw,
                                                                            geglu or pixel_shuffle, out) \
             and not _edge_narrow_eligible(x, x2, p, up2, pad_t, pad_l, out_hw, geglu or pixel_shuffle or emb is not None):
@@ -195,6 +196,20 @@
             if tile >= 0:
                 TILE_TABLE[key] = tile
 
+    if up2 and phases is not None and UP2_PHASES and splits == 1 and x.dtype == torch.bfloat16 and gn is None \
+            and x2 is None and emb is None and res is None and ln_rows is None and d.out_mode == 0 and not d.out_f32 \
+            and (p.kh, p.kw, p.stride, pt, pl) == (3, 3, 1, 1, 1) and (ho, wo) == (2 * h, 2 * w) \
+            and phases.weight.dtype == torch.bfloat16 and phases.cout == p.cout and phases.wld == 4 * c0:
+        dp = ConvDesc.from_buffer_copy(d)
+        dp.weight, dp.wld = phases.weight.data_ptr(), phases.wld
+        key = tile_key(n * h * w, c0, 0, phases, 2, 0, False, False, act, odt)
+        ptile = TILE_TABLE.get(key, -1) if FORCE_TILE is None else FORCE_TILE
+        ptag = ("conv", 2.0 * n * h * w * 4 * c0 * p.cout * 4,
+                (n, h, w, c0, c1, p.cout, p.kh, p.stride, False, 2, d.out_mode))
+        if _launch_soft(ptag, "rdeic_conv2d_up2_phases", C.byref(dp), phases.weight.stride(0), ptile, stream_ptr()):
+            if part is not None:
+                _attach_gn_part(out, part, d.gn_hw)
+            return out
     tag = ("conv", flops, (n, h, w, c0, c1, p.cout, p.kh, p.stride, gn is not None, int(up2), d.out_mode))
     if splits > 1:
         ws = _splitk_workspace(splits * n * ho * wo * p.cout, x.device)
@@ -226,6 +241,7 @@
 
 
 AUTOTUNE = False
+UP2_PHASES = True
 FORCE_TILE: Optional[int] = None
 GEGLU_FUSED = True
 TILE_CANDIDATES = (0, 1, 3, 4, 6, 8, 10)
@@ -235,7 +251,7 @@
                                                                      "conv_tiles.json")
 
 
-def tile_key(m: int, c0: int, c1: int, p: "ConvParams", up2: bool, out_mode: int, res: bool, emb: bool, act: int,
+def tile_key(m: int, c0: int, c1: int, p: "ConvParams", up2, out_mode: int, res: bool, emb: bool, act: int,
              odt) -> str:
     return (f"m{m}:c{c0}+{c1}:o{p.cout}:k{p.kh}x{p.kw}:s{p.stride}:up{int(up2)}:om{out_mode}:"
             f"r{int(res)}:e{int(emb)}:a{act}:{'f32' if odt == torch.float32 else 'bf16'}")
@@ -377,6 +393,19 @@
     record_profile(tag, ev0, ev1)
 
 
+def _launch_soft(tag, name: str, *args) -> bool:
+    if PROFILE is None:
+        return _lib.call_soft(name, *args, tag=tag)
+    ev0 = torch.cuda.Event(enable_timing=True)
+    ev1 = torch.cuda.Event(enable_timing=True)
+    ev0.record()
+    if not _lib.call_soft(name, *args, tag=tag):
+        return False
+    ev1.record()
+    record_profile(tag, ev0, ev1)
+    return True
+
+
 def record_profile(tag, ev0, ev1):
     kind, work, meta = tag
     if kind == "conv":
@@ -468,6 +497,14 @@
 
 COUNT_HALO_CONV, COUNT_GN_APPLY, COUNT_LAYERNORM, COUNT_HALO_SMALL, COUNT_LN_FUSED, COUNT_SPLITK, COUNT_EDGE, \
     COUNT_GN_PARTS_APPLY = 0, 1, 2, 3, 4, 5, 6, 7
+
+
+def set_up2_phases(on: bool) -> bool:
+    global UP2_PHASES
+    prev = UP2_PHASES
+    UP2_PHASES = bool(on)
+    _lib.load().rdeic_set_conv_option(11, int(UP2_PHASES))
+    return prev
 
 
 def launch_count(kind: int) -> int:
diff --git a/rdeic_amd/params.py b/rdeic_amd/params.py
--- a/rdeic_amd/params.py
+++ b/rdeic_amd/params.py
@@ -6,6 +6,15 @@
 
 from . import ops
 from . import weights as W
+
+
+def fold_up2_phases(w: torch.Tensor, dtype=torch.float32) -> torch.Tensor:
+    cout, cin, kh, kw = w.shape
+    if (kh, kw) != (3, 3):
+        raise ValueError("the phase fold is for 3x3 convs")
+    r = torch.tensor([[[1, 0, 0], [0, 1, 1]], [[1, 1, 0], [0, 0, 1]]], dtype=torch.float64, device=w.device)
+    f = torch.einsum("ayk,oikl,bxl->aboyxi", r, w.double(), r)
+    return f.reshape(4, cout, 4 * cin).to(dtype).contiguous()
 
 
 class ParamStore:
@@ -87,6 +96,20 @@
             self._packed[key] = p
         return p
 
+    def conv_up2_phases(self, prefix: str) -> Optional[ops.ConvParams]:
+        w = self.t[prefix + ".weight"]
+        if self.compute_dtype != torch.bfloat16 or w.dim() != 4 or tuple(w.shape[2:]) != (3, 3) or w.shape[1] % 64:
+            return None
+        key = (prefix, "up2_phases")
+        p = self._packed.get(key)
+        if p is None:
+            b = self.t.get(prefix + ".bias")
+            f = fold_up2_phases(w).to(torch.bfloat16).contiguous()
+            p = ops.ConvParams(f, 4 * w.shape[1], self.conv(prefix).bias if b is not None else None, w.shape[0],
+                               w.shape[1], 2, 2, 1, 1)
+            self._packed[key] = p
+        return p
+
     def conv_split_pad(self, prefix: str, c0: int, c0_pad: int, dtype=None) -> ops.ConvParams:
         dtype = dtype or self.compute_dtype
         key = (prefix, "split_pad", c0, c0_pad, dtype)
diff --git a/rdeic_amd/unet.py b/rdeic_amd/unet.py
--- a/rdeic_amd/unet.py
+++ b/rdeic_amd/unet.py
@@ -254,7 +254,7 @@
             elif isinstance(layer, Down):
                 x = ops.conv2d(x, s.conv(layer.prefix, stride=2, pad=1), stats=st)
             elif isinstance(layer, Up):
-                x = ops.conv2d(x, s.conv(layer.prefix), up2=True, stats=st)
+                x = ops.conv2d(x, s.conv(layer.prefix), up2=True, stats=st, phases=s.conv_up2_phases(layer.prefix))
             else:
                 raise TypeError(layer)
         return x
diff --git a/rdeic_amd/vae.py b/rdeic_amd/vae.py
--- a/rdeic_amd/vae.py
+++ b/rdeic_amd/vae.py
@@ -147,6 +147,6 @@
             for blk in lvl:
                 h = self.resnet(blk, h)
             if up is not None:
-                h = ops.conv2d(h, s.conv(up), up2=True, stats=True)
+                h = ops.conv2d(h, s.conv(up), up2=True, stats=True, phases=s.conv_up2_phases(up))
         ab = ops.group_norm_ab(h, s.get(d + "norm_out.weight"), s.get(d + "norm_out.bias"), 32, GN_EPS)
         return ops.conv2d(h, s.conv(d + "conv_out"), gn=ab, gn_silu=True, out_f32=out_f32)
```
